# elasticdeeplearning/trainingjob-operator

Measured on AMD Instinct MI355X. Metric: tokens_per_sec_llama3_8b, higher is better.
Workload: dtype bf16; 1 GPU; model=llama3-8b, global_batch=4, seq_len=4096, parallelism=dp1, micro_batch=2, grad_accum=2, checkpoint_activations=False

## Files before the change

trainingjob_operator_amd/ops/attention.py:

```python
from __future__ import annotations

import math
import os
from typing import Optional

import torch

from . import native


def _supported(q: torch.Tensor, k: torch.Tensor) -> bool:
    B, H, S, D = q.shape
    HKV = k.shape[1]
    return (q.dtype == torch.bfloat16 and D == 128
            and (S % 256 == 0 or (S % 64 == 0 and HKV == H))
            and q.stride(-1) == 1 and k.stride(-1) == 1
            and H % HKV == 0)


def _run_fwd(q, k, v, scale):
    B, H, S, D = q.shape
    HKV = k.shape[1]
    lib = native.load(require=True)
    out = torch.empty(B, H, S, D, dtype=torch.bfloat16, device=q.device)
    lse = torch.empty(B, H, S, dtype=torch.float32, device=q.device)
    rc = lib.attn_fwd(
        native.stream_ptr(), q.data_ptr(), k.data_ptr(), v.data_ptr(),
        out.data_ptr(), lse.data_ptr(),
        q.stride(0), q.stride(1), q.stride(2),
        k.stride(0), k.stride(1), k.stride(2),
        v.stride(0), v.stride(1), v.stride(2),
        B, H, HKV, S, scale)
    native.check_rc(rc, "attn_fwd", f"B={B} H={H} HKV={HKV} S={S}")
    return out, lse


class _NativeFlashAttention(torch.autograd.Function):
    @staticmethod
    def forward(ctx, q, k, v, scale):
        out, lse = _run_fwd(q, k, v, scale)
        ctx.save_for_backward(q, k, v, out, lse)
        ctx.scale = scale
        return out

    @staticmethod
    def backward(ctx, gout):
        q, k, v, out, lse = ctx.saved_tensors
        B, H, S, D = q.shape
        if S % 256 == 0 and os.environ.get("AITJ_ATTN_BWD") != "aten":
            return (*_native_backward(q, k, v, out, lse, gout, ctx.scale),
                    None)
        philox = torch.empty(0, dtype=torch.int64, device=q.device)
        dq, dk, dv = torch.ops.aten._scaled_dot_product_flash_attention_backward(
            gout.contiguous(), q, k, v, out, lse,
            None, None, S, S, 0.0, True,
            philox, philox, scale=ctx.scale)
        return dq, dk, dv, None


def _native_backward(q, k, v, out, lse, gout, scale):
    B, H, S, D = q.shape
    HKV = k.shape[1]
    lib = native.load(require=True)
    dout = gout.contiguous()
    delta = torch.empty(B, H, S, dtype=torch.float32, device=q.device)
    dq = torch.empty(B, H, S, D, dtype=torch.bfloat16, device=q.device)
    dk = torch.empty(B, HKV, S, D, dtype=torch.bfloat16, device=q.device)
    dv = torch.empty(B, HKV, S, D, dtype=torch.bfloat16, device=q.device)
    rc = lib.attn_bwd(
        native.stream_ptr(), q.data_ptr(), k.data_ptr(), v.data_ptr(),
        out.data_ptr(), dout.data_ptr(), lse.data_ptr(), delta.data_ptr(),
        dq.data_ptr(), dk.data_ptr(), dv.data_ptr(),
        q.stride(0), q.stride(1), q.stride(2),
        k.stride(0), k.stride(1), k.stride(2),
        v.stride(0), v.stride(1), v.stride(2),
        B, H, HKV, S, scale)
    native.check_rc(rc, "attn_bwd", f"B={B} H={H} HKV={HKV} S={S}")
    return dq, dk, dv


def flash_attention(q: torch.Tensor, k: torch.Tensor, v: torch.Tensor,
                    scale: Optional[float] = None) -> torch.Tensor:
    if scale is None:
        scale = 1.0 / math.sqrt(q.shape[-1])
    assert _supported(q, k), (
        f"native flash attention needs bf16, D=128, S%256==0 (or S%64==0 "
        f"with equal head counts), d-contiguous strides; got {q.shape} "
        f"{q.dtype} kv={k.shape}")
    return _NativeFlashAttention.apply(q, k, v, scale)



def _bhsd_strides(row: int, D: int, S: int):
    return (S * row, D, row)


def _rope_packed(lib, x, out, inv_freq, n_tokens, n_rot, x_row, out_row,
                 S, D, sign):
    assert inv_freq.device == x.device and inv_freq.dtype == torch.float32, (
        f"inv_freq must be fp32 on {x.device}, got "
        f"{inv_freq.dtype}@{inv_freq.device}")
    rc = lib.rope_packed(native.stream_ptr(), x.data_ptr(), out.data_ptr(),
                         inv_freq.data_ptr(), n_tokens, n_rot, x_row,
                         out_row, S, D, sign)
    native.check_rc(rc, "rope_packed", f"D={D} n_rot={n_rot} row={x_row}")


class _PackedRopeAttention(torch.autograd.Function):

    @staticmethod
    def forward(ctx, qkv, inv_freq, n_heads, n_kv_heads, scale):
        B, S, W = qkv.shape
        D = 128
        H, HKV = n_heads, n_kv_heads
        assert W == (H + 2 * HKV) * D
        qkv = qkv.contiguous()
        lib = native.load(require=True)
        R = (H + HKV) * D
        rot = torch.empty(B, S, R, dtype=torch.bfloat16, device=qkv.device)
        _rope_packed(lib, qkv, rot, inv_freq, B * S, H + HKV, W, R, S, D, 1.0)
        o = torch.empty(B, S, H * D, dtype=torch.bfloat16, device=qkv.device)
        lse = torch.empty(B, H, S, dtype=torch.float32, device=qkv.device)
        esz = qkv.element_size()
        st = native.stride_array(
            _bhsd_strides(R, D, S), _bhsd_strides(R, D, S),
            _bhsd_strides(W, D, S), _bhsd_strides(H * D, D, S))
        rc = lib.attn_fwd_strided(
            native.stream_ptr(), rot.data_ptr(),
            rot.data_ptr() + H * D * esz,
            qkv.data_ptr() + (H + HKV) * D * esz,
            o.data_ptr(), lse.data_ptr(), st, B, H, HKV, S, scale)
        native.check_rc(rc, "attn_fwd_strided", f"B={B} H={H} HKV={HKV} S={S}")
        ctx.save_for_backward(rot, qkv, o, lse, inv_freq)
        ctx.dims = (B, S, H, HKV, D)
        ctx.scale = scale
        return o

    @staticmethod
    def backward(ctx, gout):
        rot, qkv, o, lse, inv_freq = ctx.saved_tensors
        B, S, H, HKV, D = ctx.dims
        W, R = (H + 2 * HKV) * D, (H + HKV) * D
        lib = native.load(require=True)
        dout = gout if gout.is_contiguous() else gout.contiguous()
        delta = torch.empty(B, H, S, dtype=torch.float32, device=qkv.device)
        dqkv = torch.empty(B, S, W, dtype=torch.bfloat16, device=qkv.device)
        esz = qkv.element_size()
        rs, ws, os_ = (_bhsd_strides(R, D, S), _bhsd_strides(W, D, S),
                       _bhsd_strides(H * D, D, S))
        st = native.stride_array(rs, rs, ws, os_, os_, ws, ws, ws)
        rc = lib.attn_bwd_strided(
            native.stream_ptr(), rot.data_ptr(),
            rot.data_ptr() + H * D * esz,
            qkv.data_ptr() + (H + HKV) * D * esz,
            o.data_ptr(), dout.data_ptr(), lse.data_ptr(), delta.data_ptr(),
            dqkv.data_ptr(), dqkv.data_ptr() + H * D * esz,
            dqkv.data_ptr() + (H + HKV) * D * esz,
            st, B, H, HKV, S, ctx.scale)
        native.check_rc(rc, "attn_bwd_strided", f"B={B} H={H} HKV={HKV} S={S}")
        _rope_packed(lib, dqkv, dqkv, inv_freq, B * S, H + HKV, W, W, S, D,
                     -1.0)
        return dqkv, None, None, None, None


def packed_supported(qkv: torch.Tensor, n_heads: int, n_kv_heads: int) -> bool:
    return (qkv.is_cuda and qkv.dtype == torch.bfloat16 and qkv.dim() == 3
            and qkv.shape[1] % 256 == 0 and n_heads % n_kv_heads == 0
            and qkv.shape[2] == (n_heads + 2 * n_kv_heads) * 128)


def unpacked_rope_attention(qkv, inv_freq, n_heads, n_kv_heads, scale=None):
    from .functional import apply_rope
    B, S, W = qkv.shape
    D = W // (n_heads + 2 * n_kv_heads)
    q, k, v = qkv.split([n_heads * D, n_kv_heads * D, n_kv_heads * D], dim=-1)
    q = q.reshape(B, S, n_heads, D).contiguous()
    k = k.reshape(B, S, n_kv_heads, D).contiguous()
    v = v.reshape(B, S, n_kv_heads, D)
    q = apply_rope(q, inv_freq, S).transpose(1, 2)
    k = apply_rope(k, inv_freq, S).transpose(1, 2)
    v = v.transpose(1, 2)
    if qkv.is_cuda and _supported(q, k):
        o = flash_attention(q, k, v, scale)
    else:
        o = torch.nn.functional.scaled_dot_product_attention(
            q, k, v, is_causal=True, scale=scale,
            enable_gqa=n_heads != n_kv_heads)
    return o.transpose(1, 2).reshape(B, S, n_heads * D)


def packed_rope_attention(qkv: torch.Tensor, inv_freq: torch.Tensor,
                          n_heads: int, n_kv_heads: int,
                          scale: Optional[float] = None) -> torch.Tensor:
    if packed_supported(qkv, n_heads, n_kv_heads):
        if scale is None:
            scale = 1.0 / math.sqrt(128)
        return _PackedRopeAttention.apply(qkv, inv_freq, n_heads, n_kv_heads,
                                          scale)
    return unpacked_rope_attention(qkv, inv_freq, n_heads, n_kv_heads, scale)


def flash_attention_fwd_only(q, k, v, scale=None):
    if scale is None:
        scale = 1.0 / math.sqrt(q.shape[-1])
    return _run_fwd(q, k, v, scale)


def flash_attention_fwd_nw8(q, k, v, scale=None):
    if scale is None:
        scale = 1.0 / math.sqrt(q.shape[-1])
    B, H, S, D = q.shape
    HKV = k.shape[1]
    lib = native.load(require=True)
    out = torch.empty(B, H, S, D, dtype=torch.bfloat16, device=q.device)
    lse = torch.empty(B, H, S, dtype=torch.float32, device=q.device)
    rc = lib.attn_fwd_nw8(
        native.stream_ptr(), q.data_ptr(), k.data_ptr(), v.data_ptr(),
        out.data_ptr(), lse.data_ptr(),
        q.stride(0), q.stride(1), q.stride(2),
        k.stride(0), k.stride(1), k.stride(2),
        v.stride(0), v.stride(1), v.stride(2),
        B, H, HKV, S, scale)
    native.check_rc(rc, "attn_fwd_nw8", f"B={B} H={H} S={S}")
    return out, lse


def flash_attention_fwd_v7(q, k, v, scale=None):
    if scale is None:
        scale = 1.0 / math.sqrt(q.shape[-1])
    B, H, S, D = q.shape
    HKV = k.shape[1]
    lib = native.load(require=True)
    out = torch.empty(B, H, S, D, dtype=torch.bfloat16, device=q.device)
    lse = torch.empty(B, H, S, dtype=torch.float32, device=q.device)
    rc = lib.attn_fwd_v7(
        native.stream_ptr(), q.data_ptr(), k.data_ptr(), v.data_ptr(),
        out.data_ptr(), lse.data_ptr(),
        q.stride(0), q.stride(1), q.stride(2),
        k.stride(0), k.stride(1), k.stride(2),
        v.stride(0), v.stride(1), v.stride(2),
        B, H, HKV, S, scale)
    native.check_rc(rc, "attn_fwd_v7", f"B={B} H={H} S={S}")
    return out, lse


def flash_attention_fwd_v5(q, k, v, scale=None):
    if scale is None:
        scale = 1.0 / math.sqrt(q.shape[-1])
    B, H, S, D = q.shape
    lib = native.load(require=True)
    out = torch.empty(B, H, S, D, dtype=torch.bfloat16, device=q.device)
    lse = torch.empty(B, H, S, dtype=torch.float32, device=q.device)
    rc = lib.attn_fwd_v5(
        native.stream_ptr(), q.data_ptr(), k.data_ptr(), v.data_ptr(),
        out.data_ptr(), lse.data_ptr(),
        q.stride(0), q.stride(1), q.stride(2),
        k.stride(0), k.stride(1), k.stride(2),
        v.stride(0), v.stride(1), v.stride(2),
        B, H, S, scale)
    native.check_rc(rc, "attn_fwd_v5", f"B={B} H={H} S={S}")
    return out, lse



def block_supported(q: torch.Tensor, k: torch.Tensor) -> bool:
    if q.dim() != 4 or k.dim() != 4:
        return False
    B, H, S, D = q.shape
    HKV = k.shape[1]
    return (q.is_cuda and k.is_cuda and q.dtype == torch.bfloat16
            and k.dtype == torch.bfloat16 and D == 128 and k.shape[-1] == 128
            and S % 256 == 0 and k.shape[2] == S and H % HKV == 0
            and q.stride(-1) == 1 and k.stride(-1) == 1)


def _tri(t: torch.Tensor):
    assert t.stride(-1) == 1, f"last stride must be 1, got {t.stride()}"
    return (t.stride(0), t.stride(1), t.stride(2))


def _block_dims(q, k, v, op):
    assert block_supported(q, k) and v.shape == k.shape \
        and v.dtype == q.dtype and v.is_cuda, (
            f"{op} needs GPU bf16 [B,H,S,128] / [B,HKV,S,128] with "
            f"S%256==0; got q {tuple(q.shape)} {q.dtype} "
            f"kv {tuple(k.shape)} {tuple(v.shape)}")
    B, H, S, _ = q.shape
    return B, H, k.shape[1], S


def flash_attention_block_fwd(q, k, v, causal: bool,
                              scale: Optional[float] = None):
    if scale is None:
        scale = 1.0 / math.sqrt(q.shape[-1])
    B, H, HKV, S = _block_dims(q, k, v, "flash_attention_block_fwd")
    lib = native.load(require=True)
    out = torch.empty(B, H, S, 128, dtype=torch.bfloat16, device=q.device)
    lse = torch.empty(B, H, S, dtype=torch.float32, device=q.device)
    st = native.stride_array(_tri(q), _tri(k), _tri(v), _tri(out))
    rc = lib.attn_block_fwd(
        native.stream_ptr(), q.data_ptr(), k.data_ptr(), v.data_ptr(),
        out.data_ptr(), lse.data_ptr(), st, B, H, HKV, S, scale,
        1 if causal else 0)
    native.check_rc(rc, "attn_block_fwd", f"B={B} H={H} HKV={HKV} S={S}")
    return out, lse


def flash_attention_delta(out: torch.Tensor,
                          dout: torch.Tensor) -> torch.Tensor:
    assert (out.is_cuda and out.dtype == torch.bfloat16
            and dout.dtype == torch.bfloat16 and out.shape == dout.shape
            and out.dim() == 4 and out.shape[-1] == 128
            and out.shape[2] % 16 == 0), (out.shape, out.dtype, dout.dtype)
    B, H, S, _ = out.shape
    lib = native.load(require=True)
    delta = torch.empty(B, H, S, dtype=torch.float32, device=out.device)
    st = native.stride_array(_tri(out), _tri(dout))
    rc = lib.attn_delta(native.stream_ptr(), out.data_ptr(), dout.data_ptr(),
                        delta.data_ptr(), st, B, H, S)
    native.check_rc(rc, "attn_delta", f"B={B} H={H} S={S}")
    return delta


def flash_attention_block_bwd(q, k, v, dout, lse, delta, causal: bool,
                              scale: Optional[float] = None):
    if scale is None:
        scale = 1.0 / math.sqrt(q.shape[-1])
    B, H, HKV, S = _block_dims(q, k, v, "flash_attention_block_bwd")
    assert dout.shape == q.shape and dout.dtype == torch.bfloat16
    assert lse.shape == (B, H, S) and delta.shape == (B, H, S)
    assert lse.dtype == torch.float32 and delta.dtype == torch.float32
    lib = native.load(require=True)
    if dout.stride(-1) != 1:
        dout = dout.contiguous()
    lse, delta = lse.contiguous(), delta.contiguous()
    dq = torch.empty(B, H, S, 128, dtype=torch.bfloat16, device=q.device)
    dk = torch.empty(B, HKV, S, 128, dtype=torch.bfloat16, device=q.device)
    dv = torch.empty(B, HKV, S, 128, dtype=torch.bfloat16, device=q.device)
    st = native.stride_array(_tri(q), _tri(k), _tri(v), _tri(dout),
                             _tri(dq), _tri(dk), _tri(dv))
    rc = lib.attn_block_bwd(
        native.stream_ptr(), q.data_ptr(), k.data_ptr(), v.data_ptr(),
        dout.data_ptr(), lse.data_ptr(), delta.data_ptr(),
        dq.data_ptr(), dk.data_ptr(), dv.data_ptr(), st,
        B, H, HKV, S, scale, 1 if causal else 0)
    native.check_rc(rc, "attn_block_bwd", f"B={B} H={H} HKV={HKV} S={S}")
    return dq, dk, dv


def attn_merge_(o_acc, lse_acc, o_blk, lse_blk) -> None:
    B, H, S, D = o_acc.shape
    assert (o_acc.is_cuda and D == 128 and o_acc.dtype == torch.float32
            and lse_acc.dtype == torch.float32
            and lse_blk.dtype == torch.float32
            and o_blk.dtype == torch.bfloat16
            and o_acc.is_contiguous() and lse_acc.is_contiguous()
            and o_blk.shape == o_acc.shape
            and lse_acc.shape == (B, H, S) and lse_blk.shape == (B, H, S)), (
        o_acc.shape, o_acc.dtype, o_blk.shape, o_blk.dtype, lse_acc.shape,
        lse_blk.shape)
    lib = native.load(require=True)
    lse_blk = lse_blk.contiguous()
    st = native.stride_array(_tri(o_blk))
    rc = lib.attn_merge(native.stream_ptr(), o_acc.data_ptr(),
                        lse_acc.data_ptr(), o_blk.data_ptr(),
                        lse_blk.data_ptr(), st, B, H, S)
    native.check_rc(rc, "attn_merge", f"B={B} H={H} S={S}")
```

trainingjob_operator_amd/ops/hip/attention.hip:

```cpp

#include <hip/hip_runtime.h>
#include <hip/hip_bf16.h>
#include <cstdint>

typedef unsigned short u16;
typedef unsigned int u32;
typedef __attribute__((ext_vector_type(8))) __bf16 bf16x8;
typedef __attribute__((ext_vector_type(4))) float f32x4;

#define ATTN_BM 64
#define ATTN_BN 64
#define ATTN_D 128
#define ATTN_WAVES 4
__device__ __forceinline__ u16 attn_f2bf(float f) {
  __hip_bfloat16_raw r = __float2bfloat16(f);
  return r.x;
}

__device__ __forceinline__ float bf2f_(u16 b) {
  union { u32 u; float f; } c;
  c.u = ((u32)b) << 16;
  return c.f;
}

__device__ __forceinline__ int k_byte(int row, int col_elem) {
  return (row * ATTN_D * 2 + col_elem * 2) ^ ((row & 15) << 4);
}

#define VT_PITCH_B 144
__device__ __forceinline__ int vt_byte(int d, int kv) {
  const int m = d >> 3;
  return (d * VT_PITCH_B + kv * 2) ^
         ((((m & 7) | (((m >> 1) & 1) << 3))) << 4);
}

__device__ __forceinline__ int p_byte(int row, int col_elem) {
  return (row * ATTN_BN * 2 + col_elem * 2) ^ ((row & 7) << 4);
}

__global__ __launch_bounds__(256) void attn_fwd_kernel(
    const u16* __restrict__ q, const u16* __restrict__ k,
    const u16* __restrict__ v, u16* __restrict__ out,
    float* __restrict__ lse,
    long q_sb, long q_sh, long q_ss,
    long k_sb, long k_sh, long k_ss,
    long v_sb, long v_sh, long v_ss,
    int n_heads, int S, float scale) {
  const int qb = blockIdx.x;
  const int h = blockIdx.y;
  const int b = blockIdx.z;
  const int wid = threadIdx.x >> 6;
  const int lane = threadIdx.x & 63;
  const int low = lane & 15;
  const int kg = lane >> 4;

  __shared__ u16 ldsK[ATTN_BN * ATTN_D];
  __shared__ u16 ldsV[ATTN_D * (VT_PITCH_B / 2) + 128];
  __shared__ u16 ldsP[ATTN_WAVES][16 * ATTN_BN];

  const u16* qbase = q + (long)b * q_sb + (long)h * q_sh
                     + (long)(qb * ATTN_BM) * q_ss;
  union { bf16x8 v; uint4 u; } qfrag[4];
#pragma unroll
  for (int ks = 0; ks < 4; ++ks) {
    qfrag[ks].u = *reinterpret_cast<const uint4*>(
        qbase + (long)(wid * 16 + low) * q_ss + ks * 32 + kg * 8);
  }

  float m_run[4], l_run[4];
  float oacc[8][4];
#pragma unroll
  for (int r = 0; r < 4; ++r) { m_run[r] = -INFINITY; l_run[r] = 0.f; }
#pragma unroll
  for (int ct = 0; ct < 8; ++ct)
#pragma unroll
    for (int r = 0; r < 4; ++r) oacc[ct][r] = 0.f;

  const u16* kbase = k + (long)b * k_sb + (long)h * k_sh;
  const u16* vbase = v + (long)b * v_sb + (long)h * v_sh;
  const int kv_end = (qb + 1) * ATTN_BM;
  char* ldsKb = reinterpret_cast<char*>(ldsK);
  char* ldsVb = reinterpret_cast<char*>(ldsV);
  char* ldsPb = reinterpret_cast<char*>(ldsP[wid]);

  for (int kv0 = 0; kv0 < kv_end; kv0 += ATTN_BN) {
#pragma unroll
    for (int t = 0; t < 4; ++t) {
      const int idx = t * 256 + threadIdx.x;
      const int r = idx >> 4;
      const int c8 = (idx & 15) * 8;
      *reinterpret_cast<uint4*>(&ldsKb[k_byte(r, c8)]) =
          *reinterpret_cast<const uint4*>(
              kbase + (long)(kv0 + r) * k_ss + c8);
      union { uint4 u; u16 h[8]; } vv;
      vv.u = *reinterpret_cast<const uint4*>(
          vbase + (long)(kv0 + r) * v_ss + c8);
#pragma unroll
      for (int j = 0; j < 8; ++j)
        *reinterpret_cast<u16*>(&ldsVb[vt_byte(c8 + j, r)]) = vv.h[j];
    }
    __syncthreads();

    f32x4 sacc[4];
#pragma unroll
    for (int ct = 0; ct < 4; ++ct) {
      f32x4 acc = {0.f, 0.f, 0.f, 0.f};
#pragma unroll
      for (int ks = 0; ks < 4; ++ks) {
        bf16x8 bfrag = *reinterpret_cast<const bf16x8*>(
            &ldsKb[k_byte(ct * 16 + low, ks * 32 + kg * 8)]);
        acc = __builtin_amdgcn_mfma_f32_16x16x32_bf16(qfrag[ks].v, bfrag,
                                                      acc, 0, 0, 0);
      }
      sacc[ct] = acc;
    }

    const int qrow0 = qb * ATTN_BM + wid * 16 + kg * 4;
    float mx[4], alpha[4], psum[4];
#pragma unroll
    for (int r = 0; r < 4; ++r) {
      mx[r] = -INFINITY;
#pragma unroll
      for (int ct = 0; ct < 4; ++ct) {
        const int col = kv0 + ct * 16 + low;
        float s = sacc[ct][r] * scale;
        if (col > qrow0 + r) s = -INFINITY;
        sacc[ct][r] = s;
        mx[r] = fmaxf(mx[r], s);
      }
#pragma unroll
      for (int off = 1; off < 16; off <<= 1)
        mx[r] = fmaxf(mx[r], __shfl_xor(mx[r], off, 64));
      const float mnew = fmaxf(m_run[r], mx[r]);
      alpha[r] = (m_run[r] == -INFINITY) ? 0.f : __expf(m_run[r] - mnew);
      m_run[r] = mnew;
      psum[r] = 0.f;
#pragma unroll
      for (int ct = 0; ct < 4; ++ct) {
        const float p = (sacc[ct][r] == -INFINITY)
                            ? 0.f : __expf(sacc[ct][r] - mnew);
        sacc[ct][r] = p;
        psum[r] += p;
        *reinterpret_cast<u16*>(
            &ldsPb[p_byte(kg * 4 + r, ct * 16 + low)]) = attn_f2bf(p);
      }
#pragma unroll
      for (int off = 1; off < 16; off <<= 1)
        psum[r] += __shfl_xor(psum[r], off, 64);
      l_run[r] = l_run[r] * alpha[r] + psum[r];
#pragma unroll
      for (int ct2 = 0; ct2 < 8; ++ct2) oacc[ct2][r] *= alpha[r];
    }
    __syncthreads();

#pragma unroll
    for (int ct2 = 0; ct2 < 8; ++ct2) {
      f32x4 acc = {oacc[ct2][0], oacc[ct2][1], oacc[ct2][2], oacc[ct2][3]};
#pragma unroll
      for (int ks2 = 0; ks2 < 2; ++ks2) {
        bf16x8 afrag = *reinterpret_cast<const bf16x8*>(
            &ldsPb[p_byte(low, ks2 * 32 + kg * 8)]);
        bf16x8 bfrag = *reinterpret_cast<const bf16x8*>(
            &ldsVb[vt_byte(ct2 * 16 + low, ks2 * 32 + kg * 8)]);
        acc = __builtin_amdgcn_mfma_f32_16x16x32_bf16(afrag, bfrag, acc,
                                                      0, 0, 0);
      }
#pragma unroll
      for (int r = 0; r < 4; ++r) oacc[ct2][r] = acc[r];
    }
    __syncthreads();
  }

  u16* obase = out + (((long)b * n_heads + h) * S + qb * ATTN_BM
                      + wid * 16) * ATTN_D;
#pragma unroll
  for (int r = 0; r < 4; ++r) {
    const float inv_l = 1.0f / l_run[r];
#pragma unroll
    for (int ct2 = 0; ct2 < 8; ++ct2) {
      obase[(long)(kg * 4 + r) * ATTN_D + ct2 * 16 + low] =
          attn_f2bf(oacc[ct2][r] * inv_l);
    }
  }
  if (low == 0) {
    float* lbase = lse + ((long)b * n_heads + h) * S + qb * ATTN_BM
                   + wid * 16 + kg * 4;
#pragma unroll
    for (int r = 0; r < 4; ++r) lbase[r] = m_run[r] + __logf(l_run[r]);
  }
}


typedef __attribute__((ext_vector_type(16))) float f32x16;

#define V6_BM 256
#define V6_QBLK 32
#define V6_BN 64
#define V6_K_U16 (V6_BN * ATTN_D)
#define V6_V_U16 (ATTN_D * (VT_PITCH_B / 2) + 128)
#define V6_BUF_U16 (V6_K_U16 + V6_V_U16)

__device__ __forceinline__ unsigned cvt_pk_bf16(float lo, float hi) {
  unsigned r;
  asm("v_cvt_pk_bf16_f32 %0, %1, %2" : "=v"(r) : "v"(lo), "v"(hi));
  return r;
}

__device__ __forceinline__ float exp2_raw(float x) {
  float r;
  asm("v_exp_f32 %0, %1" : "=v"(r) : "v"(x));
  return r;
}

__device__ __forceinline__ void v7_wait_vmcnt4() {
  asm volatile("s_waitcnt vmcnt(4)" ::: "memory");
}
__device__ __forceinline__ void v7_wait_vmcnt0() {
  asm volatile("s_waitcnt vmcnt(0)" ::: "memory");
}
__device__ __forceinline__ void v7_barrier() {
  asm volatile("s_waitcnt lgkmcnt(0)" ::: "memory");
  __builtin_amdgcn_s_barrier();
}

#define V7_RING 3


template <int NW>
__global__ __launch_bounds__(NW * 64) void attn_fwd_v6_kernel(
    const u16* __restrict__ q, const u16* __restrict__ k,
    const u16* __restrict__ v, u16* __restrict__ out,
    float* __restrict__ lse,
    long q_sb, long q_sh, long q_ss,
    long k_sb, long k_sh, long k_ss,
    long v_sb, long v_sh, long v_ss,
    int n_heads, int gqa_group, int S, float scale2) {
  constexpr int NT = NW * 64;
  constexpr int BM = NW * 32;
  constexpr int KP = 1024 / NT;
  constexpr int VU = 512 / NT;
  const int qb = gridDim.x - 1 - blockIdx.x;
  const int h = blockIdx.y;
  const int b = blockIdx.z;
  const int hkv = h / gqa_group;
  const int tid = threadIdx.x;
  const int wid = tid >> 6;
  const int lane = tid & 63;
  const int low = lane & 31;
  const int hi = lane >> 5;

  __shared__ __attribute__((aligned(16))) u16 lds[2][V6_BUF_U16];

  const int q0w = qb * BM + wid * V6_QBLK;
  const int qrow = q0w + low;

  union F8 { bf16x8 v; uint4 u; u16 h[8]; };
  const u16* qptr = q + (long)b * q_sb + (long)h * q_sh + (long)qrow * q_ss;
  F8 qf[8];
#pragma unroll
  for (int kc = 0; kc < 8; ++kc)
    qf[kc].u = *reinterpret_cast<const uint4*>(qptr + kc * 16 + hi * 8);

  f32x16 oacc[4];
#pragma unroll
  for (int ds = 0; ds < 4; ++ds)
#pragma unroll
    for (int r = 0; r < 16; ++r) oacc[ds][r] = 0.f;
  float m_run = -INFINITY, l_run = 0.f;

  const u16* kbase = k + (long)b * k_sb + (long)hkv * k_sh;
  const u16* vbase = v + (long)b * v_sb + (long)hkv * v_sh;
  const int n_tiles = (qb * BM + BM) / V6_BN;

  char* lds0 = reinterpret_cast<char*>(&lds[0][0]);
  char* lds1 = reinterpret_cast<char*>(&lds[1][0]);
  const int VOFF = V6_K_U16 * 2;

  const u16* kgp[KP];
  const u16* vgp[2 * VU];
#pragma unroll
  for (int i = 0; i < KP; ++i) {
    const int idx = i * NT + tid;
    const int L = idx * 16;
    const int kr = L >> 8;
    const int kin = (((L & 255) ^ ((kr & 15) << 4)) >> 1);
    kgp[i] = kbase + (long)kr * k_ss + kin;
  }
#pragma unroll
  for (int u = 0; u < VU; ++u) {
    const int unit = u * NT + tid;
    const int rp2 = (unit >> 4) * 2;
    const int c8 = (unit & 15) * 8;
#pragma unroll
    for (int i = 0; i < 2; ++i)
      vgp[u * 2 + i] = vbase + (long)(rp2 + i) * v_ss + c8;
  }
  const long kstep = (long)V6_BN * k_ss;
  const long vstep = (long)V6_BN * v_ss;
  const int wu64 = __builtin_amdgcn_readfirstlane(tid >> 6);

  uint4 vst[2 * VU];
#define V6_GLDS_K(BUFI)                                                     \
  _Pragma("unroll")                                                         \
  for (int i = 0; i < KP; ++i) {                                            \
    __builtin_amdgcn_global_load_lds(                                       \
        (const u32*)kgp[i], (u32*)&lds[BUFI][(i * NT + wu64 * 64) * 8],     \
        16, 0, 0);                                                          \
    kgp[i] += kstep;                                                        \
  }
#define V6_LOAD_V()                                                         \
  _Pragma("unroll")                                                         \
  for (int i = 0; i < 2 * VU; ++i) {                                        \
    vst[i] = *reinterpret_cast<const uint4*>(vgp[i]);                       \
    vgp[i] += vstep;                                                        \
  }
#define V6_WRITE_V(BUF)                                                     \
  _Pragma("unroll")                                                         \
  for (int u = 0; u < VU; ++u) {                                            \
    const int unit_ = u * NT + tid;                                         \
    const int rp2_ = (unit_ >> 4) * 2;                                      \
    const int c8_ = (unit_ & 15) * 8;                                       \
    union { uint4 u4; u16 h[8]; } va_, vb_;                                 \
    va_.u4 = vst[u * 2];                                                    \
    vb_.u4 = vst[u * 2 + 1];                                                \
    _Pragma("unroll")                                                       \
    for (int j = 0; j < 8; ++j) {                                           \
      const u32 pair_ = (u32)va_.h[j] | ((u32)vb_.h[j] << 16);              \
      *reinterpret_cast<u32*>(&(BUF)[VOFF + vt_byte(c8_ + j, rp2_)]) = pair_; \
    }                                                                       \
  }

  V6_GLDS_K(0)
  V6_LOAD_V()
  V6_WRITE_V(lds0)
  __syncthreads();

  if (NW == 8 && __builtin_amdgcn_readfirstlane(threadIdx.x) >= NT / 2)
    __builtin_amdgcn_s_setprio(1);

  int cur = 0;
  for (int t = 0; t < n_tiles; ++t) {
    const int kv0 = t * V6_BN;
    const bool have_next = (t + 1) < n_tiles;
    if (have_next) { V6_GLDS_K(cur ^ 1) V6_LOAD_V() }

    char* kb = cur ? lds1 : lds0;
    char* vbuf = kb + VOFF;
    const bool active = kv0 <= q0w + V6_QBLK - 1;
    const bool need_mask = kv0 + V6_BN > q0w;

    f32x16 s0, s1;
    union PF { bf16x8 v; unsigned u[4]; } pa[4];
    float pm = -INFINITY;
    if (active) {
#pragma unroll
      for (int r = 0; r < 16; ++r) { s0[r] = 0.f; s1[r] = 0.f; }
#pragma unroll
      for (int kc = 0; kc < 8; ++kc) {
        bf16x8 a0 = *reinterpret_cast<const bf16x8*>(
            &kb[k_byte(low, kc * 16 + hi * 8)]);
        s0 = __builtin_amdgcn_mfma_f32_32x32x16_bf16(a0, qf[kc].v, s0, 0, 0, 0);
        bf16x8 a1 = *reinterpret_cast<const bf16x8*>(
            &kb[k_byte(32 + low, kc * 16 + hi * 8)]);
        s1 = __builtin_amdgcn_mfma_f32_32x32x16_bf16(a1, qf[kc].v, s1, 0, 0, 0);
      }
      if (need_mask) {
#pragma unroll
        for (int r = 0; r < 16; ++r) {
          const int kvr = kv0 + (r & 3) + 8 * (r >> 2) + 4 * hi;
          float x0 = s0[r] * scale2;
          if (kvr > qrow) x0 = -1e30f;
          s0[r] = x0;
          float x1 = s1[r] * scale2;
          if (kvr + 32 > qrow) x1 = -1e30f;
          s1[r] = x1;
          pm = fmaxf(pm, fmaxf(x0, x1));
        }
      } else {
#pragma unroll
        for (int r = 0; r < 16; ++r) {
          s0[r] *= scale2;
          s1[r] *= scale2;
          pm = fmaxf(pm, fmaxf(s0[r], s1[r]));
        }
      }
      pm = fmaxf(pm, __shfl_xor(pm, 32, 64));
    }
    if (have_next) {
      char* nb = cur ? lds0 : lds1;
      V6_WRITE_V(nb)
    }
    if (active) {
      if (!__all(pm - m_run <= 8.0f)) {
        const float mn = fmaxf(m_run, pm);
        const float alpha = (m_run == -INFINITY) ? 0.f : exp2_raw(m_run - mn);
        m_run = mn;
        l_run *= alpha;
#pragma unroll
        for (int ds = 0; ds < 4; ++ds)
#pragma unroll
          for (int r = 0; r < 16; ++r) oacc[ds][r] *= alpha;
      }
      float psum = 0.f;
#pragma unroll
      for (int r = 0; r < 16; ++r) {
        const float p0 = exp2_raw(s0[r] - m_run);
        const float p1 = exp2_raw(s1[r] - m_run);
        s0[r] = p0;
        s1[r] = p1;
        psum += p0 + p1;
      }
      psum += __shfl_xor(psum, 32, 64);
      l_run += psum;

#pragma unroll
      for (int sub = 0; sub < 2; ++sub) {
#pragma unroll
        for (int cc = 0; cc < 2; ++cc) {
          const int pb = cc * 8;
          unsigned a0, b0, a1, b1;
          if (sub == 0) {
            a0 = cvt_pk_bf16(s0[pb + 0], s0[pb + 1]);
            b0 = cvt_pk_bf16(s0[pb + 4], s0[pb + 5]);
            a1 = cvt_pk_bf16(s0[pb + 2], s0[pb + 3]);
            b1 = cvt_pk_bf16(s0[pb + 6], s0[pb + 7]);
          } else {
            a0 = cvt_pk_bf16(s1[pb + 0], s1[pb + 1]);
            b0 = cvt_pk_bf16(s1[pb + 4], s1[pb + 5]);
            a1 = cvt_pk_bf16(s1[pb + 2], s1[pb + 3]);
            b1 = cvt_pk_bf16(s1[pb + 6], s1[pb + 7]);
          }
          auto r02 = __builtin_amdgcn_permlane32_swap(a0, b0, false, false);
          auto r13 = __builtin_amdgcn_permlane32_swap(a1, b1, false, false);
          PF f;
          f.u[0] = r02[0];
          f.u[1] = r13[0];
          f.u[2] = r02[1];
          f.u[3] = r13[1];
          pa[sub * 2 + cc] = f;
        }
      }

#pragma unroll
      for (int c = 0; c < 4; ++c) {
#pragma unroll
        for (int ds = 0; ds < 4; ++ds) {
          bf16x8 vf = *reinterpret_cast<const bf16x8*>(
              &vbuf[vt_byte(ds * 32 + low, c * 16 + hi * 8)]);
          oacc[ds] = __builtin_amdgcn_mfma_f32_32x32x16_bf16(
              vf, pa[c].v, oacc[ds], 0, 0, 0);
        }
      }
    }
    __syncthreads();
    cur ^= 1;
  }

  const float inv_l = 1.0f / l_run;
  u16* orow = out + (((long)b * n_heads + h) * S + qrow) * ATTN_D;
#pragma unroll
  for (int ds = 0; ds < 4; ++ds) {
#pragma unroll
    for (int g = 0; g < 4; ++g) {
      const int d0 = 8 * g + 4 * hi + 32 * ds;
      const unsigned w0 = cvt_pk_bf16(oacc[ds][4 * g + 0] * inv_l,
                                      oacc[ds][4 * g + 1] * inv_l);
      const unsigned w1 = cvt_pk_bf16(oacc[ds][4 * g + 2] * inv_l,
                                      oacc[ds][4 * g + 3] * inv_l);
      uint2 wv;
      wv.x = w0;
      wv.y = w1;
      *reinterpret_cast<uint2*>(orow + d0) = wv;
    }
  }
  if (hi == 0)
    lse[((long)b * n_heads + h) * S + qrow] =
        m_run * 0.6931471805599453f + __logf(l_run);
}

template <bool CAUSAL>
__global__ __launch_bounds__(512) void attn_fwd_v7_kernel(
    const u16* __restrict__ q, const u16* __restrict__ k,
    const u16* __restrict__ v, u16* __restrict__ out,
    float* __restrict__ lse,
    long q_sb, long q_sh, long q_ss,
    long k_sb, long k_sh, long k_ss,
    long v_sb, long v_sh, long v_ss,
    long o_sb, long o_sh, long o_ss,
    int n_heads, int gqa_group, int S, float scale2);

static inline bool attn_strides_ok(const long* st, int n) {
  for (int i = 0; i < n; ++i)
    if (st[i] < 0 || st[i] % 8 != 0) return false;
  return true;
}

static void launch_fwd_v7(void* stream, const void* q, const void* k,
                          const void* v, void* out, void* lse,
                          long q_sb, long q_sh, long q_ss,
                          long k_sb, long k_sh, long k_ss,
                          long v_sb, long v_sh, long v_ss,
                          long o_sb, long o_sh, long o_ss,
                          int batch, int n_heads, int n_kv_heads, int S,
                          float scale, bool causal = true) {
  const float scale2 = scale * 1.4426950408889634f;
  dim3 grid(S / 256, n_heads, batch), block(512);
  hipLaunchKernelGGL(causal ? attn_fwd_v7_kernel<true>
                            : attn_fwd_v7_kernel<false>, grid, block, 0,
                     reinterpret_cast<hipStream_t>(stream),
                     (const u16*)q, (const u16*)k, (const u16*)v,
                     (u16*)out, (float*)lse, q_sb, q_sh, q_ss,
                     k_sb, k_sh, k_ss, v_sb, v_sh, v_ss,
                     o_sb, o_sh, o_ss, n_heads,
                     n_heads / n_kv_heads, S, scale2);
}

extern "C" int attn_fwd(void* stream, const void* q, const void* k,
                        const void* v, void* out, void* lse,
                        long q_sb, long q_sh, long q_ss,
                        long k_sb, long k_sh, long k_ss,
                        long v_sb, long v_sh, long v_ss,
                        int batch, int n_heads, int n_kv_heads, int S,
                        float scale) {
  if (S <= 0 || n_heads <= 0 || batch <= 0 || n_kv_heads <= 0 ||
      n_heads % n_kv_heads != 0)
    return -1;
  if (S % 128 == 0) {
    const float scale2 = scale * 1.4426950408889634f;
    if (S % 256 == 0) {
      launch_fwd_v7(stream, q, k, v, out, lse, q_sb, q_sh, q_ss,
                    k_sb, k_sh, k_ss, v_sb, v_sh, v_ss,
                    (long)n_heads * S * ATTN_D, (long)S * ATTN_D, ATTN_D,
                    batch, n_heads, n_kv_heads, S, scale);
      return 0;
    }
    dim3 grid(S / 128, n_heads, batch), block(256);
    hipLaunchKernelGGL((attn_fwd_v6_kernel<4>), grid, block, 0,
                       reinterpret_cast<hipStream_t>(stream),
                       (const u16*)q, (const u16*)k, (const u16*)v, (u16*)out,
                       (float*)lse, q_sb, q_sh, q_ss, k_sb, k_sh, k_ss,
                       v_sb, v_sh, v_ss, n_heads, n_heads / n_kv_heads, S,
                       scale2);
    return 0;
  }
  if (S % ATTN_BM != 0 || n_kv_heads != n_heads) return -1;
  dim3 grid(S / ATTN_BM, n_heads, batch), block(256);
  hipLaunchKernelGGL(attn_fwd_kernel, grid, block, 0,
                     reinterpret_cast<hipStream_t>(stream),
                     (const u16*)q, (const u16*)k, (const u16*)v, (u16*)out,
                     (float*)lse, q_sb, q_sh, q_ss, k_sb, k_sh, k_ss,
                     v_sb, v_sh, v_ss, n_heads, S, scale);
  return 0;
}

extern "C" int attn_fwd_nw8(void* stream, const void* q, const void* k,
                            const void* v, void* out, void* lse,
                            long q_sb, long q_sh, long q_ss,
                            long k_sb, long k_sh, long k_ss,
                            long v_sb, long v_sh, long v_ss,
                            int batch, int n_heads, int n_kv_heads, int S,
                            float scale) {
  if (S <= 0 || S % 256 != 0 || n_heads % n_kv_heads != 0) return -1;
  dim3 grid(S / 256, n_heads, batch), block(512);
  const float scale2 = scale * 1.4426950408889634f;
  hipLaunchKernelGGL((attn_fwd_v6_kernel<8>), grid, block, 0,
                     reinterpret_cast<hipStream_t>(stream),
                     (const u16*)q, (const u16*)k, (const u16*)v, (u16*)out,
                     (float*)lse, q_sb, q_sh, q_ss, k_sb, k_sh, k_ss,
                     v_sb, v_sh, v_ss, n_heads, n_heads / n_kv_heads, S,
                     scale2);
  return 0;
}

extern "C" int attn_fwd_v5(void* stream, const void* q, const void* k,
                           const void* v, void* out, void* lse,
                           long q_sb, long q_sh, long q_ss,
                           long k_sb, long k_sh, long k_ss,
                           long v_sb, long v_sh, long v_ss,
                           int batch, int n_heads, int S, float scale) {
  if (S <= 0 || S % ATTN_BM != 0 || n_heads <= 0 || batch <= 0) return -1;
  dim3 grid(S / ATTN_BM, n_heads, batch), block(256);
  hipLaunchKernelGGL(attn_fwd_kernel, grid, block, 0,
                     reinterpret_cast<hipStream_t>(stream),
                     (const u16*)q, (const u16*)k, (const u16*)v, (u16*)out,
                     (float*)lse, q_sb, q_sh, q_ss, k_sb, k_sh, k_ss,
                     v_sb, v_sh, v_ss, n_heads, S, scale);
  return 0;
}


__global__ __launch_bounds__(256) void attn_delta_kernel(
    const u16* __restrict__ dout, const u16* __restrict__ o,
    float* __restrict__ delta,
    long do_sb, long do_sh, long do_ss,
    long o_sb, long o_sh, long o_ss,
    int n_heads, int S) {
  const int s = blockIdx.x * 16 + (threadIdx.x >> 4);
  const int h = blockIdx.y;
  const int bi = blockIdx.z;
  if (s >= S) return;
  const long row = ((long)bi * n_heads + h) * S + s;
  const int e8 = (threadIdx.x & 15) * 8;
  union { uint4 u; u16 h[8]; } a, b;
  a.u = *reinterpret_cast<const uint4*>(
      dout + (long)bi * do_sb + (long)h * do_sh + (long)s * do_ss + e8);
  b.u = *reinterpret_cast<const uint4*>(
      o + (long)bi * o_sb + (long)h * o_sh + (long)s * o_ss + e8);
  float acc = 0.f;
#pragma unroll
  for (int j = 0; j < 8; ++j)
    acc += bf2f_(a.h[j]) * bf2f_(b.h[j]);
#pragma unroll
  for (int off = 1; off < 16; off <<= 1) acc += __shfl_xor(acc, off, 64);
  if ((threadIdx.x & 15) == 0) delta[row] = acc;
}


#define BQ_K_U16 (V6_BN * ATTN_D)
#define BQ_KT_U16 (ATTN_D * (VT_PITCH_B / 2) + 128)
#define BQ_V_U16 (V6_BN * ATTN_D)
#define BQ_BUF_U16 (BQ_K_U16 + BQ_KT_U16 + BQ_V_U16)

template <bool CAUSAL>
__global__ __launch_bounds__(512) void attn_bwd_dq_kernel(
    const u16* __restrict__ q, const u16* __restrict__ k,
    const u16* __restrict__ v, const u16* __restrict__ dout,
    const float* __restrict__ lse, const float* __restrict__ delta,
    u16* __restrict__ dq,
    long q_sb, long q_sh, long q_ss,
    long k_sb, long k_sh, long k_ss,
    long v_sb, long v_sh, long v_ss,
    long do_sb, long do_sh, long do_ss,
    long dq_sb, long dq_sh, long dq_ss,
    int n_heads, int gqa_group, int S, float scale) {
  constexpr int NT = 512;
  const int qb = gridDim.x - 1 - blockIdx.x;
  const int h = blockIdx.y;
  const int b = blockIdx.z;
  const int hkv = h / gqa_group;
  const int tid = threadIdx.x;
  const int wid = tid >> 6;
  const int lane = tid & 63;
  const int low = lane & 31;
  const int hi = lane >> 5;
  const float scale2 = scale * 1.4426950408889634f;

  __shared__ __attribute__((aligned(16))) u16
      lds[V7_RING * 2 * V6_K_U16 + 2 * V6_V_U16];
#define DQ_K(SLOT) (&lds[(SLOT) * V6_K_U16])
#define DQ_VR(SLOT) (&lds[(V7_RING + (SLOT)) * V6_K_U16])
#define DQ_KT(P) (reinterpret_cast<char*>(&lds[2 * V7_RING * V6_K_U16]) \
                  + (P) * (V6_V_U16 * 2))

  const int q0w = qb * 256 + wid * 32;
  const int qrow = q0w + low;

  union F8 { bf16x8 v; uint4 u; u16 h[8]; };
  const u16* qptr = q + (long)b * q_sb + (long)h * q_sh + (long)qrow * q_ss;
  const u16* doptr = dout + (long)b * do_sb + (long)h * do_sh
                     + (long)qrow * do_ss;
  F8 qf[8], dof[8];
#pragma unroll
  for (int kc = 0; kc < 8; ++kc) {
    qf[kc].u = *reinterpret_cast<const uint4*>(qptr + kc * 16 + hi * 8);
    dof[kc].u = *reinterpret_cast<const uint4*>(doptr + kc * 16 + hi * 8);
  }
  const long lrow = ((long)b * n_heads + h) * S + qrow;
  const float lse2 = lse[lrow] * 1.4426950408889634f;
  const float dlt = delta[lrow];

  f32x16 dqacc[4];
#pragma unroll
  for (int ds = 0; ds < 4; ++ds)
#pragma unroll
    for (int r = 0; r < 16; ++r) dqacc[ds][r] = 0.f;

  const u16* kbase = k + (long)b * k_sb + (long)hkv * k_sh;
  const u16* vbase = v + (long)b * v_sb + (long)hkv * v_sh;
  const int n_tiles = CAUSAL ? (qb + 1) * 4 : S / V6_BN;

  const u16* kgp[2];
  const u16* vgp[2];
#pragma unroll
  for (int i = 0; i < 2; ++i) {
    const int L = (tid & ~63) * 32 + i * 1024 + (tid & 63) * 16;
    const int kr = L >> 8;
    const int kin = (((L & 255) ^ ((kr & 15) << 4)) >> 1);
    kgp[i] = kbase + (long)kr * k_ss + kin;
    vgp[i] = vbase + (long)kr * v_ss + kin;
  }
  const long kstep = (long)V6_BN * k_ss;
  const long vstep = (long)V6_BN * v_ss;
  const int lslot = (tid & ~63) * 16;

#define DQ_GLDS(SLOT)                                                       \
  _Pragma("unroll")                                                         \
  for (int i = 0; i < 2; ++i) {                                             \
    __builtin_amdgcn_global_load_lds(                                       \
        (const u32*)kgp[i], (u32*)&DQ_K(SLOT)[i * 512 + lslot],          \
        16, 0, 0);                                                          \
    kgp[i] += kstep;                                                        \
    __builtin_amdgcn_global_load_lds(                                       \
        (const u32*)vgp[i], (u32*)&DQ_VR(SLOT)[i * 512 + lslot],         \
        16, 0, 0);                                                          \
    vgp[i] += vstep;                                                        \
  }

  const int t_rp2 = (tid >> 4) * 2;
  const int t_c8 = (tid & 15) * 8;
#define DQ_TRANSPOSE(SRCSLOT, DST)                                          \
  {                                                                         \
    const char* srcb = reinterpret_cast<const char*>(DQ_K(SRCSLOT));        \
    union { uint4 u4; u16 h[8]; } va_, vb_;                                 \
    va_.u4 = *reinterpret_cast<const uint4*>(&srcb[k_byte(t_rp2, t_c8)]);   \
    vb_.u4 = *reinterpret_cast<const uint4*>(                               \
        &srcb[k_byte(t_rp2 + 1, t_c8)]);                                    \
    _Pragma("unroll")                                                       \
    for (int j = 0; j < 8; ++j) {                                           \
      const u32 pair_ = (u32)va_.h[j] | ((u32)vb_.h[j] << 16);              \
      *reinterpret_cast<u32*>(&(DST)[vt_byte(t_c8 + j, t_rp2)]) = pair_;    \
    }                                                                       \
  }

  DQ_GLDS(0)
  if (n_tiles > 1) DQ_GLDS(1)
  if (n_tiles > 1) v7_wait_vmcnt4(); else v7_wait_vmcnt0();
  v7_barrier();
  DQ_TRANSPOSE(0, DQ_KT(0))
  v7_barrier();

  for (int t = 0; t < n_tiles; ++t) {
    const int kv0 = t * V6_BN;
    const bool have2 = (t + 2) < n_tiles;
    if (have2) DQ_GLDS((t + 2) % V7_RING)

    char* kb = reinterpret_cast<char*>(DQ_K(t % V7_RING));
    char* vb = reinterpret_cast<char*>(DQ_VR(t % V7_RING));
    char* ktb = DQ_KT(t & 1);
    const bool active = !CAUSAL || kv0 <= q0w + 31;
    const bool need_mask = CAUSAL && kv0 + V6_BN > q0w;

    union PF { bf16x8 v; unsigned u[4]; } pds[4];
    if (active) {
#pragma unroll
      for (int sub = 0; sub < 2; ++sub) {
        f32x16 sx, dp;
#pragma unroll
        for (int r = 0; r < 16; ++r) { sx[r] = 0.f; dp[r] = 0.f; }
#pragma unroll
        for (int kc = 0; kc < 8; ++kc) {
          bf16x8 a = *reinterpret_cast<const bf16x8*>(
              &kb[k_byte(sub * 32 + low, kc * 16 + hi * 8)]);
          sx = __builtin_amdgcn_mfma_f32_32x32x16_bf16(a, qf[kc].v, sx,
                                                       0, 0, 0);
          bf16x8 a2 = *reinterpret_cast<const bf16x8*>(
              &vb[k_byte(sub * 32 + low, kc * 16 + hi * 8)]);
          dp = __builtin_amdgcn_mfma_f32_32x32x16_bf16(a2, dof[kc].v, dp,
                                                       0, 0, 0);
        }
#pragma unroll
        for (int r = 0; r < 16; ++r) {
          float x = sx[r] * scale2 - lse2;
          if (need_mask) {
            const int kvr = kv0 + sub * 32 + (r & 3) + 8 * (r >> 2) + 4 * hi;
            if (kvr > qrow) x = -1e30f;
          }
          const float p = exp2_raw(x);
          sx[r] = p * (dp[r] - dlt) * scale;
        }
#pragma unroll
        for (int cc = 0; cc < 2; ++cc) {
          const int pb = cc * 8;
          unsigned a0 = cvt_pk_bf16(sx[pb + 0], sx[pb + 1]);
          unsigned b0 = cvt_pk_bf16(sx[pb + 4], sx[pb + 5]);
          unsigned a1 = cvt_pk_bf16(sx[pb + 2], sx[pb + 3]);
          unsigned b1 = cvt_pk_bf16(sx[pb + 6], sx[pb + 7]);
          auto r02 = __builtin_amdgcn_permlane32_swap(a0, b0, false, false);
          auto r13 = __builtin_amdgcn_permlane32_swap(a1, b1, false, false);
          PF f;
          f.u[0] = r02[0];
          f.u[1] = r13[0];
          f.u[2] = r02[1];
          f.u[3] = r13[1];
          pds[sub * 2 + cc] = f;
        }
      }
#pragma unroll
      for (int c = 0; c < 4; ++c) {
#pragma unroll
        for (int ds = 0; ds < 4; ++ds) {
          bf16x8 kf = *reinterpret_cast<const bf16x8*>(
              &ktb[vt_byte(ds * 32 + low, c * 16 + hi * 8)]);
          dqacc[ds] = __builtin_amdgcn_mfma_f32_32x32x16_bf16(
              kf, pds[c].v, dqacc[ds], 0, 0, 0);
        }
      }
    }
    if (t + 1 < n_tiles) {
      if (have2) v7_wait_vmcnt4(); else v7_wait_vmcnt0();
      DQ_TRANSPOSE((t + 1) % V7_RING, DQ_KT((t + 1) & 1))
    }
    v7_barrier();
  }

  u16* dqrow = dq + (long)b * dq_sb + (long)h * dq_sh + (long)qrow * dq_ss;
#pragma unroll
  for (int ds = 0; ds < 4; ++ds) {
#pragma unroll
    for (int g = 0; g < 4; ++g) {
      const int d0 = 8 * g + 4 * hi + 32 * ds;
      const unsigned w0 = cvt_pk_bf16(dqacc[ds][4 * g + 0],
                                      dqacc[ds][4 * g + 1]);
      const unsigned w1 = cvt_pk_bf16(dqacc[ds][4 * g + 2],
                                      dqacc[ds][4 * g + 3]);
      uint2 wv;
      wv.x = w0;
      wv.y = w1;
      *reinterpret_cast<uint2*>(dqrow + d0) = wv;
    }
  }
}


#define BV_Q_U16 (V6_BN * ATTN_D)
#define BV_DOT_U16 (ATTN_D * (VT_PITCH_B / 2) + 128)
#define BV_LSE_U16 128
#define BV_BUF_U16 (BV_Q_U16 + BV_DOT_U16 + BV_LSE_U16)

template <bool CAUSAL>
__global__ __launch_bounds__(512) void attn_bwd_dv_kernel(
    const u16* __restrict__ q, const u16* __restrict__ k,
    const u16* __restrict__ dout, const float* __restrict__ lse,
    u16* __restrict__ dv,
    long q_sb, long q_sh, long q_ss,
    long k_sb, long k_sh, long k_ss,
    long do_sb, long do_sh, long do_ss,
    long dv_sb, long dv_sh, long dv_ss,
    int n_heads, int n_kv_heads, int S, float scale) {
  const int kvb = blockIdx.x;
  const int hkv = blockIdx.y;
  const int b = blockIdx.z;
  const int gqa_group = n_heads / n_kv_heads;
  const int tid = threadIdx.x;
  const int wid = tid >> 6;
  const int lane = tid & 63;
  const int low = lane & 31;
  const int hi = lane >> 5;
  const float scale2 = scale * 1.4426950408889634f;

  __shared__ __attribute__((aligned(16))) u16 lds[2][BV_BUF_U16];
  char* lds0 = reinterpret_cast<char*>(&lds[0][0]);
  char* lds1 = reinterpret_cast<char*>(&lds[1][0]);
  const int DOTOFF = BV_Q_U16 * 2;
  const int LSEOFF = (BV_Q_U16 + BV_DOT_U16) * 2;

  const int kv0w = kvb * 256 + wid * 32;
  const int kvrow = kv0w + low;

  union F8 { bf16x8 v; uint4 u; u16 h[8]; };
  const u16* kptr = k + (long)b * k_sb + (long)hkv * k_sh + (long)kvrow * k_ss;
  F8 kf[8];
#pragma unroll
  for (int kc = 0; kc < 8; ++kc)
    kf[kc].u = *reinterpret_cast<const uint4*>(kptr + kc * 16 + hi * 8);

  f32x16 dvacc[4];
#pragma unroll
  for (int ds = 0; ds < 4; ++ds)
#pragma unroll
    for (int r = 0; r < 16; ++r) dvacc[ds][r] = 0.f;

  const int qt0 = CAUSAL ? kvb * 4 : 0;
  const int qtn = S / 64;
  const int wu64 = __builtin_amdgcn_readfirstlane(tid >> 6);
  uint4 dtst[2];

  for (int g = 0; g < gqa_group; ++g) {
    const int h = hkv * gqa_group + g;
    const u16* qbase = q + (long)b * q_sb + (long)h * q_sh;
    const u16* dobase = dout + (long)b * do_sb + (long)h * do_sh;
    const float* lbase = lse + ((long)b * n_heads + h) * S;

    const u16* qgp[2];
    const u16* dtp[2];
    {
      const int idx0 = tid, idx1 = 512 + tid;
      const int L0 = idx0 * 16, L1 = idx1 * 16;
      const int r0 = L0 >> 8, r1 = L1 >> 8;
      const int in0 = (((L0 & 255) ^ ((r0 & 15) << 4)) >> 1);
      const int in1 = (((L1 & 255) ^ ((r1 & 15) << 4)) >> 1);
      qgp[0] = qbase + (long)(qt0 * 64 + r0) * q_ss + in0;
      qgp[1] = qbase + (long)(qt0 * 64 + r1) * q_ss + in1;
      const int rp2 = (tid >> 4) * 2;
      const int c8 = (tid & 15) * 8;
      dtp[0] = dobase + (long)(qt0 * 64 + rp2) * do_ss + c8;
      dtp[1] = dobase + (long)(qt0 * 64 + rp2 + 1) * do_ss + c8;
    }
    const long qstep = (long)64 * q_ss;
    const long dostep = (long)64 * do_ss;

#define BV_STAGE_IN(BUFI, QT)                                               \
    {                                                                       \
      _Pragma("unroll")                                                     \
      for (int i = 0; i < 2; ++i) {                                         \
        __builtin_amdgcn_global_load_lds(                                   \
            (const u32*)qgp[i], (u32*)&lds[BUFI][(i * 512 + wu64 * 64) * 8],\
            16, 0, 0);                                                      \
        qgp[i] += qstep;                                                    \
      }                                                                     \
      dtst[0] = *reinterpret_cast<const uint4*>(dtp[0]);                    \
      dtst[1] = *reinterpret_cast<const uint4*>(dtp[1]);                    \
      dtp[0] += dostep;                                                     \
      dtp[1] += dostep;                                                     \
      if (tid < 64)                                                         \
        *reinterpret_cast<float*>(                                          \
            &lds[BUFI][LSEOFF / 2 + tid * 2]) =                             \
            lbase[(QT) * 64 + tid] * 1.4426950408889634f;                   \
    }
#define BV_WRITE_DOT(BUF)                                                   \
    {                                                                       \
      const int rp2_ = (tid >> 4) * 2;                                      \
      const int c8_ = (tid & 15) * 8;                                       \
      union { uint4 u4; u16 h[8]; } va_, vb_;                               \
      va_.u4 = dtst[0];                                                     \
      vb_.u4 = dtst[1];                                                     \
      _Pragma("unroll")                                                     \
      for (int j = 0; j < 8; ++j) {                                         \
        const u32 pair_ = (u32)va_.h[j] | ((u32)vb_.h[j] << 16);            \
        *reinterpret_cast<u32*>(&(BUF)[DOTOFF + vt_byte(c8_ + j, rp2_)]) =  \
            pair_;                                                          \
      }                                                                     \
    }

    BV_STAGE_IN(0, qt0)
    BV_WRITE_DOT(lds0)
    __syncthreads();

    int cur = 0;
    for (int qt = qt0; qt < qtn; ++qt) {
      const bool have_next = (qt + 1) < qtn;
      if (have_next) BV_STAGE_IN(cur ^ 1, qt + 1)

      char* qb_ = cur ? lds1 : lds0;
      char* dob = qb_ + DOTOFF;
      const float* lse2t = reinterpret_cast<const float*>(qb_ + LSEOFF);
      const bool active = !CAUSAL || qt * 64 + 63 >= kv0w;
      const bool need_mask = CAUSAL && qt * 64 < kv0w + 32;

      union PF { bf16x8 v; unsigned u[4]; } pf[4];
      if (active) {
#pragma unroll
        for (int sub = 0; sub < 2; ++sub) {
          f32x16 s;
#pragma unroll
          for (int r = 0; r < 16; ++r) s[r] = 0.f;
#pragma unroll
          for (int kc = 0; kc < 8; ++kc) {
            bf16x8 a = *reinterpret_cast<const bf16x8*>(
                &qb_[k_byte(sub * 32 + low, kc * 16 + hi * 8)]);
            s = __builtin_amdgcn_mfma_f32_32x32x16_bf16(a, kf[kc].v, s,
                                                        0, 0, 0);
          }
#pragma unroll
          for (int r = 0; r < 16; ++r) {
            const int qr = (r & 3) + 8 * (r >> 2) + 4 * hi;
            float x = s[r] * scale2 - lse2t[sub * 32 + qr];
            if (need_mask && qt * 64 + sub * 32 + qr < kvrow) x = -1e30f;
            s[r] = exp2_raw(x);
          }
#pragma unroll
          for (int cc = 0; cc < 2; ++cc) {
            const int pb = cc * 8;
            unsigned a0 = cvt_pk_bf16(s[pb + 0], s[pb + 1]);
            unsigned b0 = cvt_pk_bf16(s[pb + 4], s[pb + 5]);
            unsigned a1 = cvt_pk_bf16(s[pb + 2], s[pb + 3]);
            unsigned b1 = cvt_pk_bf16(s[pb + 6], s[pb + 7]);
            auto r02 = __builtin_amdgcn_permlane32_swap(a0, b0, false, false);
            auto r13 = __builtin_amdgcn_permlane32_swap(a1, b1, false, false);
            PF f;
            f.u[0] = r02[0];
            f.u[1] = r13[0];
            f.u[2] = r02[1];
            f.u[3] = r13[1];
            pf[sub * 2 + cc] = f;
          }
        }
      }
      if (have_next) {
        char* nb = cur ? lds0 : lds1;
        BV_WRITE_DOT(nb)
      }
      if (active) {
#pragma unroll
        for (int c = 0; c < 4; ++c) {
#pragma unroll
          for (int ds = 0; ds < 4; ++ds) {
            bf16x8 af = *reinterpret_cast<const bf16x8*>(
                &dob[vt_byte(ds * 32 + low, c * 16 + hi * 8)]);
            dvacc[ds] = __builtin_amdgcn_mfma_f32_32x32x16_bf16(
                af, pf[c].v, dvacc[ds], 0, 0, 0);
          }
        }
      }
      __syncthreads();
      cur ^= 1;
    }
  }

  u16* dvrow = dv + (long)b * dv_sb + (long)hkv * dv_sh + (long)kvrow * dv_ss;
#pragma unroll
  for (int ds = 0; ds < 4; ++ds) {
#pragma unroll
    for (int g = 0; g < 4; ++g) {
      const int d0 = 8 * g + 4 * hi + 32 * ds;
      const unsigned w0 = cvt_pk_bf16(dvacc[ds][4 * g + 0],
                                      dvacc[ds][4 * g + 1]);
      const unsigned w1 = cvt_pk_bf16(dvacc[ds][4 * g + 2],
                                      dvacc[ds][4 * g + 3]);
      uint2 wv;
      wv.x = w0;
      wv.y = w1;
      *reinterpret_cast<uint2*>(dvrow + d0) = wv;
    }
  }
}


#define BK_Q_U16 (V6_BN * ATTN_D)
#define BK_DO_U16 (V6_BN * ATTN_D)
#define BK_QT_U16 (ATTN_D * (VT_PITCH_B / 2) + 128)
#define BK_LSE_U16 128
#define BK_DLT_U16 128
#define BK_BUF_U16 (BK_Q_U16 + BK_DO_U16 + BK_QT_U16 + BK_LSE_U16 + BK_DLT_U16)

template <bool CAUSAL>
__global__ __launch_bounds__(512) void attn_bwd_dk_kernel(
    const u16* __restrict__ q, const u16* __restrict__ k,
    const u16* __restrict__ v, const u16* __restrict__ dout,
    const float* __restrict__ lse, const float* __restrict__ delta,
    u16* __restrict__ dk,
    long q_sb, long q_sh, long q_ss,
    long k_sb, long k_sh, long k_ss,
    long v_sb, long v_sh, long v_ss,
    long do_sb, long do_sh, long do_ss,
    long dk_sb, long dk_sh, long dk_ss,
    int n_heads, int n_kv_heads, int S, float scale) {
  const int kvb = blockIdx.x;
  const int hkv = blockIdx.y;
  const int b = blockIdx.z;
  const int gqa_group = n_heads / n_kv_heads;
  const int tid = threadIdx.x;
  const int wid = tid >> 6;
  const int lane = tid & 63;
  const int low = lane & 31;
  const int hi = lane >> 5;
  const float scale2 = scale * 1.4426950408889634f;

  __shared__ __attribute__((aligned(16))) u16 lds[2][BK_BUF_U16];
  char* lds0 = reinterpret_cast<char*>(&lds[0][0]);
  char* lds1 = reinterpret_cast<char*>(&lds[1][0]);
  const int DOOFF = BK_Q_U16 * 2;
  const int QTOFF = (BK_Q_U16 + BK_DO_U16) * 2;
  const int LSEOFF = (BK_Q_U16 + BK_DO_U16 + BK_QT_U16) * 2;
  const int DLTOFF = LSEOFF + BK_LSE_U16 * 2;

  const int kv0w = kvb * 256 + wid * 32;
  const int kvrow = kv0w + low;

  union F8 { bf16x8 v; uint4 u; u16 h[8]; };
  const u16* kptr = k + (long)b * k_sb + (long)hkv * k_sh + (long)kvrow * k_ss;
  const u16* vptr = v + (long)b * v_sb + (long)hkv * v_sh + (long)kvrow * v_ss;
  F8 kf[8], vf[8];
#pragma unroll
  for (int kc = 0; kc < 8; ++kc) {
    kf[kc].u = *reinterpret_cast<const uint4*>(kptr + kc * 16 + hi * 8);
    vf[kc].u = *reinterpret_cast<const uint4*>(vptr + kc * 16 + hi * 8);
  }

  f32x16 dkacc[4];
#pragma unroll
  for (int ds = 0; ds < 4; ++ds)
#pragma unroll
    for (int r = 0; r < 16; ++r) dkacc[ds][r] = 0.f;

  const int qt0 = CAUSAL ? kvb * 4 : 0;
  const int qtn = S / 64;
  const int wu64 = __builtin_amdgcn_readfirstlane(tid >> 6);
  uint4 qtst[2];

  for (int g = 0; g < gqa_group; ++g) {
    const int h = hkv * gqa_group + g;
    const u16* qbase = q + (long)b * q_sb + (long)h * q_sh;
    const u16* dobase = dout + (long)b * do_sb + (long)h * do_sh;
    const float* lbase = lse + ((long)b * n_heads + h) * S;
    const float* dbase = delta + ((long)b * n_heads + h) * S;

    const u16* qgp[2];
    const u16* dgp[2];
    const u16* qtp[2];
    {
      const int idx0 = tid, idx1 = 512 + tid;
      const int L0 = idx0 * 16, L1 = idx1 * 16;
      const int r0 = L0 >> 8, r1 = L1 >> 8;
      const int in0 = (((L0 & 255) ^ ((r0 & 15) << 4)) >> 1);
      const int in1 = (((L1 & 255) ^ ((r1 & 15) << 4)) >> 1);
      qgp[0] = qbase + (long)(qt0 * 64 + r0) * q_ss + in0;
      qgp[1] = qbase + (long)(qt0 * 64 + r1) * q_ss + in1;
      dgp[0] = dobase + (long)(qt0 * 64 + r0) * do_ss + in0;
      dgp[1] = dobase + (long)(qt0 * 64 + r1) * do_ss + in1;
      const int rp2 = (tid >> 4) * 2;
      const int c8 = (tid & 15) * 8;
      qtp[0] = qbase + (long)(qt0 * 64 + rp2) * q_ss + c8;
      qtp[1] = qbase + (long)(qt0 * 64 + rp2 + 1) * q_ss + c8;
    }
    const long qstep = (long)64 * q_ss;
    const long dostep = (long)64 * do_ss;

#define BK_STAGE_IN(BUFI, QT)                                               \
    {                                                                       \
      _Pragma("unroll")                                                     \
      for (int i = 0; i < 2; ++i) {                                         \
        __builtin_amdgcn_global_load_lds(                                   \
            (const u32*)qgp[i], (u32*)&lds[BUFI][(i * 512 + wu64 * 64) * 8],\
            16, 0, 0);                                                      \
        qgp[i] += qstep;                                                    \
        __builtin_amdgcn_global_load_lds(                                   \
            (const u32*)dgp[i],                                             \
            (u32*)&lds[BUFI][DOOFF / 2 + (i * 512 + wu64 * 64) * 8],        \
            16, 0, 0);                                                      \
        dgp[i] += dostep;                                                   \
      }                                                                     \
      qtst[0] = *reinterpret_cast<const uint4*>(qtp[0]);                    \
      qtst[1] = *reinterpret_cast<const uint4*>(qtp[1]);                    \
      qtp[0] += qstep;                                                      \
      qtp[1] += qstep;                                                      \
      if (tid < 64)                                                         \
        *reinterpret_cast<float*>(&lds[BUFI][LSEOFF / 2 + tid * 2]) =       \
            lbase[(QT) * 64 + tid] * 1.4426950408889634f;                   \
      else if (tid < 128)                                                   \
        *reinterpret_cast<float*>(                                          \
            &lds[BUFI][DLTOFF / 2 + (tid - 64) * 2]) =                      \
            dbase[(QT) * 64 + tid - 64];                                    \
    }
#define BK_WRITE_QT(BUF)                                                    \
    {                                                                       \
      const int rp2_ = (tid >> 4) * 2;                                      \
      const int c8_ = (tid & 15) * 8;                                       \
      union { uint4 u4; u16 h[8]; } va_, vb_;                               \
      va_.u4 = qtst[0];                                                     \
      vb_.u4 = qtst[1];                                                     \
      _Pragma("unroll")                                                     \
      for (int j = 0; j < 8; ++j) {                                         \
        const u32 pair_ = (u32)va_.h[j] | ((u32)vb_.h[j] << 16);            \
        *reinterpret_cast<u32*>(&(BUF)[QTOFF + vt_byte(c8_ + j, rp2_)]) =   \
            pair_;                                                          \
      }                                                                     \
    }

    BK_STAGE_IN(0, qt0)
    BK_WRITE_QT(lds0)
    __syncthreads();

    int cur = 0;
    for (int qt = qt0; qt < qtn; ++qt) {
      const bool have_next = (qt + 1) < qtn;
      if (have_next) BK_STAGE_IN(cur ^ 1, qt + 1)

      char* qb_ = cur ? lds1 : lds0;
      char* dob = qb_ + DOOFF;
      char* qtb = qb_ + QTOFF;
      const float* lse2t = reinterpret_cast<const float*>(qb_ + LSEOFF);
      const float* dltt = reinterpret_cast<const float*>(qb_ + DLTOFF);
      const bool active = !CAUSAL || qt * 64 + 63 >= kv0w;
      const bool need_mask = CAUSAL && qt * 64 < kv0w + 32;

      union PF { bf16x8 v; unsigned u[4]; } pf[4];
      if (active) {
#pragma unroll
        for (int sub = 0; sub < 2; ++sub) {
          f32x16 s, dp;
#pragma unroll
          for (int r = 0; r < 16; ++r) { s[r] = 0.f; dp[r] = 0.f; }
#pragma unroll
          for (int kc = 0; kc < 8; ++kc) {
            bf16x8 a = *reinterpret_cast<const bf16x8*>(
                &qb_[k_byte(sub * 32 + low, kc * 16 + hi * 8)]);
            s = __builtin_amdgcn_mfma_f32_32x32x16_bf16(a, kf[kc].v, s,
                                                        0, 0, 0);
            bf16x8 a2 = *reinterpret_cast<const bf16x8*>(
                &dob[k_byte(sub * 32 + low, kc * 16 + hi * 8)]);
            dp = __builtin_amdgcn_mfma_f32_32x32x16_bf16(a2, vf[kc].v, dp,
                                                         0, 0, 0);
          }
#pragma unroll
          for (int r = 0; r < 16; ++r) {
            const int qr = (r & 3) + 8 * (r >> 2) + 4 * hi;
            float x = s[r] * scale2 - lse2t[sub * 32 + qr];
            if (need_mask && qt * 64 + sub * 32 + qr < kvrow) x = -1e30f;
            const float p = exp2_raw(x);
            s[r] = p * (dp[r] - dltt[sub * 32 + qr]) * scale;
          }
#pragma unroll
          for (int cc = 0; cc < 2; ++cc) {
            const int pb = cc * 8;
            unsigned a0 = cvt_pk_bf16(s[pb + 0], s[pb + 1]);
            unsigned b0 = cvt_pk_bf16(s[pb + 4], s[pb + 5]);
            unsigned a1 = cvt_pk_bf16(s[pb + 2], s[pb + 3]);
            unsigned b1 = cvt_pk_bf16(s[pb + 6], s[pb + 7]);
            auto r02 = __builtin_amdgcn_permlane32_swap(a0, b0, false, false);
            auto r13 = __builtin_amdgcn_permlane32_swap(a1, b1, false, false);
            PF f;
            f.u[0] = r02[0];
            f.u[1] = r13[0];
            f.u[2] = r02[1];
            f.u[3] = r13[1];
            pf[sub * 2 + cc] = f;
          }
        }
      }
      if (have_next) {
        char* nb = cur ? lds0 : lds1;
        BK_WRITE_QT(nb)
      }
      if (active) {
#pragma unroll
        for (int c = 0; c < 4; ++c) {
#pragma unroll
          for (int ds = 0; ds < 4; ++ds) {
            bf16x8 af = *reinterpret_cast<const bf16x8*>(
                &qtb[vt_byte(ds * 32 + low, c * 16 + hi * 8)]);
            dkacc[ds] = __builtin_amdgcn_mfma_f32_32x32x16_bf16(
                af, pf[c].v, dkacc[ds], 0, 0, 0);
          }
        }
      }
      __syncthreads();
      cur ^= 1;
    }
  }

  u16* dkrow = dk + (long)b * dk_sb + (long)hkv * dk_sh + (long)kvrow * dk_ss;
#pragma unroll
  for (int ds = 0; ds < 4; ++ds) {
#pragma unroll
    for (int g = 0; g < 4; ++g) {
      const int d0 = 8 * g + 4 * hi + 32 * ds;
      const unsigned w0 = cvt_pk_bf16(dkacc[ds][4 * g + 0],
                                      dkacc[ds][4 * g + 1]);
      const unsigned w1 = cvt_pk_bf16(dkacc[ds][4 * g + 2],
                                      dkacc[ds][4 * g + 3]);
      uint2 wv;
      wv.x = w0;
      wv.y = w1;
      *reinterpret_cast<uint2*>(dkrow + d0) = wv;
    }
  }
}




struct AttnStride { long sb, sh, ss; };

static inline AttnStride attn_dense_stride(int n_heads, int S) {
  return {(long)n_heads * S * ATTN_D, (long)S * ATTN_D, (long)ATTN_D};
}

static void launch_delta(hipStream_t st, const void* out, const void* dout,
                         void* delta, AttnStride os, AttnStride dos,
                         int batch, int n_heads, int S) {
  hipLaunchKernelGGL(attn_delta_kernel, dim3(S / 16, n_heads, batch),
                     dim3(256), 0, st,
                     (const u16*)dout, (const u16*)out, (float*)delta,
                     dos.sb, dos.sh, dos.ss, os.sb, os.sh, os.ss,
                     n_heads, S);
}

template <bool CAUSAL>
static void launch_bwd_core(hipStream_t st, const void* q, const void* k,
                            const void* v, const void* dout,
                            const void* lse, const void* delta,
                            void* dq, void* dk, void* dv,
                            AttnStride qs, AttnStride ks, AttnStride vs,
                            AttnStride dos, AttnStride dqs, AttnStride dks,
                            AttnStride dvs, int batch, int n_heads,
                            int n_kv_heads, int S, float scale) {
  {
    dim3 grid(S / 256, n_heads, batch), block(512);
    hipLaunchKernelGGL(attn_bwd_dq_kernel<CAUSAL>, grid, block, 0, st,
                       (const u16*)q, (const u16*)k, (const u16*)v,
                       (const u16*)dout, (const float*)lse,
                       (const float*)delta, (u16*)dq,
                       qs.sb, qs.sh, qs.ss, ks.sb, ks.sh, ks.ss,
                       vs.sb, vs.sh, vs.ss, dos.sb, dos.sh, dos.ss,
                       dqs.sb, dqs.sh, dqs.ss,
                       n_heads, n_heads / n_kv_heads, S, scale);
  }
  {
    dim3 grid(S / 256, n_kv_heads, batch), block(512);
    hipLaunchKernelGGL(attn_bwd_dv_kernel<CAUSAL>, grid, block, 0, st,
                       (const u16*)q, (const u16*)k, (const u16*)dout,
                       (const float*)lse, (u16*)dv,
                       qs.sb, qs.sh, qs.ss, ks.sb, ks.sh, ks.ss,
                       dos.sb, dos.sh, dos.ss, dvs.sb, dvs.sh, dvs.ss,
                       n_heads, n_kv_heads, S, scale);
    hipLaunchKernelGGL(attn_bwd_dk_kernel<CAUSAL>, grid, block, 0, st,
                       (const u16*)q, (const u16*)k, (const u16*)v,
                       (const u16*)dout, (const float*)lse,
                       (const float*)delta, (u16*)dk,
                       qs.sb, qs.sh, qs.ss, ks.sb, ks.sh, ks.ss,
                       vs.sb, vs.sh, vs.ss, dos.sb, dos.sh, dos.ss,
                       dks.sb, dks.sh, dks.ss,
                       n_heads, n_kv_heads, S, scale);
  }
}

static inline bool attn_block_shape_ok(int batch, int n_heads,
                                       int n_kv_heads, int S) {
  return S > 0 && S % 256 == 0 && n_heads > 0 && batch > 0 &&
         n_kv_heads > 0 && n_heads % n_kv_heads == 0;
}

static int launch_bwd(void* stream, const void* q, const void* k,
                      const void* v, const void* out, const void* dout,
                      const void* lse, void* delta,
                      void* dq, void* dk, void* dv,
                      AttnStride qs, AttnStride ks, AttnStride vs,
                      AttnStride os, AttnStride dos,
                      AttnStride dqs, AttnStride dks, AttnStride dvs,
                      int batch, int n_heads, int n_kv_heads, int S,
                      float scale) {
  if (!attn_block_shape_ok(batch, n_heads, n_kv_heads, S)) return -1;
  hipStream_t st = reinterpret_cast<hipStream_t>(stream);
  launch_delta(st, out, dout, delta, os, dos, batch, n_heads, S);
  launch_bwd_core<true>(st, q, k, v, dout, lse, delta, dq, dk, dv,
                        qs, ks, vs, dos, dqs, dks, dvs,
                        batch, n_heads, n_kv_heads, S, scale);
  return 0;
}

extern "C" int attn_bwd(void* stream, const void* q, const void* k,
                        const void* v, const void* out, const void* dout,
                        const void* lse, void* delta,
                        void* dq, void* dk, void* dv,
                        long q_sb, long q_sh, long q_ss,
                        long k_sb, long k_sh, long k_ss,
                        long v_sb, long v_sh, long v_ss,
                        int batch, int n_heads, int n_kv_heads, int S,
                        float scale) {
  const AttnStride dh = attn_dense_stride(n_heads, S);
  const AttnStride dkv = attn_dense_stride(n_kv_heads, S);
  return launch_bwd(stream, q, k, v, out, dout, lse, delta, dq, dk, dv,
                    {q_sb, q_sh, q_ss}, {k_sb, k_sh, k_ss},
                    {v_sb, v_sh, v_ss}, dh, dh, dh, dkv, dkv,
                    batch, n_heads, n_kv_heads, S, scale);
}

extern "C" int attn_bwd_strided(void* stream, const void* q, const void* k,
                                const void* v, const void* out,
                                const void* dout, const void* lse,
                                void* delta, void* dq, void* dk, void* dv,
                                const long* st, int batch, int n_heads,
                                int n_kv_heads, int S, float scale) {
  if (!st || !attn_strides_ok(st, 24)) return -1;
  auto tri = [st](int i) {
    return AttnStride{st[3 * i], st[3 * i + 1], st[3 * i + 2]};
  };
  return launch_bwd(stream, q, k, v, out, dout, lse, delta, dq, dk, dv,
                    tri(0), tri(1), tri(2), tri(3), tri(4), tri(5), tri(6),
                    tri(7), batch, n_heads, n_kv_heads, S, scale);
}


template <bool CAUSAL>
__global__ __launch_bounds__(512) void attn_fwd_v7_kernel(
    const u16* __restrict__ q, const u16* __restrict__ k,
    const u16* __restrict__ v, u16* __restrict__ out,
    float* __restrict__ lse,
    long q_sb, long q_sh, long q_ss,
    long k_sb, long k_sh, long k_ss,
    long v_sb, long v_sh, long v_ss,
    long o_sb, long o_sh, long o_ss,
    int n_heads, int gqa_group, int S, float scale2) {
  constexpr int NT = 512;
  const int qb = gridDim.x - 1 - blockIdx.x;
  const int h = blockIdx.y;
  const int b = blockIdx.z;
  const int hkv = h / gqa_group;
  const int tid = threadIdx.x;
  const int wid = tid >> 6;
  const int lane = tid & 63;
  const int low = lane & 31;
  const int hi = lane >> 5;

  __shared__ __attribute__((aligned(16))) u16
      lds[V7_RING * 2 * V6_K_U16 + 2 * V6_V_U16];
#define LDSK(SLOT) (&lds[(SLOT) * V6_K_U16])
#define LDSVR(SLOT) (&lds[(V7_RING + (SLOT)) * V6_K_U16])
#define LDSVT(P) (reinterpret_cast<char*>(&lds[2 * V7_RING * V6_K_U16]) \
                  + (P) * (V6_V_U16 * 2))

  const int q0w = qb * 256 + wid * 32;
  const int qrow = q0w + low;

  union F8 { bf16x8 v; uint4 u; u16 h[8]; };
  const u16* qptr = q + (long)b * q_sb + (long)h * q_sh + (long)qrow * q_ss;
  F8 qf[8];
#pragma unroll
  for (int kc = 0; kc < 8; ++kc)
    qf[kc].u = *reinterpret_cast<const uint4*>(qptr + kc * 16 + hi * 8);

  f32x16 oacc[4];
#pragma unroll
  for (int ds = 0; ds < 4; ++ds)
#pragma unroll
    for (int r = 0; r < 16; ++r) oacc[ds][r] = 0.f;
  float m_run = -INFINITY, l_run = 0.f;

  const u16* kbase = k + (long)b * k_sb + (long)hkv * k_sh;
  const u16* vbase = v + (long)b * v_sb + (long)hkv * v_sh;
  const int n_tiles = CAUSAL ? (qb + 1) * 4 : S / V6_BN;

  const u16* kgp[2];
  const u16* vgp[2];
#pragma unroll
  for (int i = 0; i < 2; ++i) {
    const int L = (tid & ~63) * 32 + i * 1024 + (tid & 63) * 16;
    const int kr = L >> 8;
    const int kin = (((L & 255) ^ ((kr & 15) << 4)) >> 1);
    kgp[i] = kbase + (long)kr * k_ss + kin;
    vgp[i] = vbase + (long)kr * v_ss + kin;
  }
  const long kstep = (long)V6_BN * k_ss;
  const long vstep = (long)V6_BN * v_ss;
  const int lslot = (tid & ~63) * 16;

#define V7_GLDS(SLOT)                                                       \
  _Pragma("unroll")                                                         \
  for (int i = 0; i < 2; ++i) {                                             \
    __builtin_amdgcn_global_load_lds(                                       \
        (const u32*)kgp[i], (u32*)&LDSK(SLOT)[i * 512 + lslot],          \
        16, 0, 0);                                                          \
    kgp[i] += kstep;                                                        \
    __builtin_amdgcn_global_load_lds(                                       \
        (const u32*)vgp[i], (u32*)&LDSVR(SLOT)[i * 512 + lslot],         \
        16, 0, 0);                                                          \
    vgp[i] += vstep;                                                        \
  }

  const int t_rp2 = (tid >> 4) * 2;
  const int t_c8 = (tid & 15) * 8;
#define V7_TRANSPOSE(SRCSLOT, DST)                                          \
  {                                                                         \
    const char* srcb = reinterpret_cast<const char*>(LDSVR(SRCSLOT));       \
    union { uint4 u4; u16 h[8]; } va_, vb_;                                 \
    va_.u4 = *reinterpret_cast<const uint4*>(&srcb[k_byte(t_rp2, t_c8)]);   \
    vb_.u4 = *reinterpret_cast<const uint4*>(                               \
        &srcb[k_byte(t_rp2 + 1, t_c8)]);                                    \
    _Pragma("unroll")                                                       \
    for (int j = 0; j < 8; ++j) {                                           \
      const u32 pair_ = (u32)va_.h[j] | ((u32)vb_.h[j] << 16);              \
      *reinterpret_cast<u32*>(&(DST)[vt_byte(t_c8 + j, t_rp2)]) = pair_;    \
    }                                                                       \
  }

  V7_GLDS(0)
  if (n_tiles > 1) V7_GLDS(1)
  if (n_tiles > 1) v7_wait_vmcnt4(); else v7_wait_vmcnt0();
  v7_barrier();
  V7_TRANSPOSE(0, LDSVT(0))
  v7_barrier();

  for (int t = 0; t < n_tiles; ++t) {
    const int kv0 = t * V6_BN;
    const bool have2 = (t + 2) < n_tiles;
    if (have2) V7_GLDS((t + 2) % V7_RING)

    char* kb = reinterpret_cast<char*>(LDSK(t % V7_RING));
    char* vtb = LDSVT(t & 1);
    const bool active = !CAUSAL || kv0 <= q0w + 31;
    const bool need_mask = CAUSAL && kv0 + V6_BN > q0w;

    f32x16 s0, s1;
    union PF { bf16x8 v; unsigned u[4]; } pa[4];
    float pm = -INFINITY;
    if (active) {
#pragma unroll
      for (int r = 0; r < 16; ++r) { s0[r] = 0.f; s1[r] = 0.f; }
#pragma unroll
      for (int kc = 0; kc < 8; ++kc) {
        bf16x8 a0 = *reinterpret_cast<const bf16x8*>(
            &kb[k_byte(low, kc * 16 + hi * 8)]);
        s0 = __builtin_amdgcn_mfma_f32_32x32x16_bf16(a0, qf[kc].v, s0, 0, 0, 0);
        bf16x8 a1 = *reinterpret_cast<const bf16x8*>(
            &kb[k_byte(32 + low, kc * 16 + hi * 8)]);
        s1 = __builtin_amdgcn_mfma_f32_32x32x16_bf16(a1, qf[kc].v, s1, 0, 0, 0);
      }
      if (need_mask) {
#pragma unroll
        for (int r = 0; r < 16; ++r) {
          const int kvr = kv0 + (r & 3) + 8 * (r >> 2) + 4 * hi;
          float x0 = s0[r] * scale2;
          if (kvr > qrow) x0 = -1e30f;
          s0[r] = x0;
          float x1 = s1[r] * scale2;
          if (kvr + 32 > qrow) x1 = -1e30f;
          s1[r] = x1;
          pm = fmaxf(pm, fmaxf(x0, x1));
        }
      } else {
#pragma unroll
        for (int r = 0; r < 16; ++r) {
          s0[r] *= scale2;
          s1[r] *= scale2;
          pm = fmaxf(pm, fmaxf(s0[r], s1[r]));
        }
      }
      pm = fmaxf(pm, __shfl_xor(pm, 32, 64));

      if (!__all(pm - m_run <= 8.0f)) {
        const float mn = fmaxf(m_run, pm);
        const float alpha = (m_run == -INFINITY) ? 0.f : exp2_raw(m_run - mn);
        m_run = mn;
        l_run *= alpha;
#pragma unroll
        for (int ds = 0; ds < 4; ++ds)
#pragma unroll
          for (int r = 0; r < 16; ++r) oacc[ds][r] *= alpha;
      }
      float psum = 0.f;
#pragma unroll
      for (int r = 0; r < 16; ++r) {
        const float p0 = exp2_raw(s0[r] - m_run);
        const float p1 = exp2_raw(s1[r] - m_run);
        s0[r] = p0;
        s1[r] = p1;
        psum += p0 + p1;
      }
      psum += __shfl_xor(psum, 32, 64);
      l_run += psum;

#pragma unroll
      for (int sub = 0; sub < 2; ++sub) {
#pragma unroll
        for (int cc = 0; cc < 2; ++cc) {
          const int pb = cc * 8;
          unsigned a0, b0, a1, b1;
          if (sub == 0) {
            a0 = cvt_pk_bf16(s0[pb + 0], s0[pb + 1]);
            b0 = cvt_pk_bf16(s0[pb + 4], s0[pb + 5]);
            a1 = cvt_pk_bf16(s0[pb + 2], s0[pb + 3]);
            b1 = cvt_pk_bf16(s0[pb + 6], s0[pb + 7]);
          } else {
            a0 = cvt_pk_bf16(s1[pb + 0], s1[pb + 1]);
            b0 = cvt_pk_bf16(s1[pb + 4], s1[pb + 5]);
            a1 = cvt_pk_bf16(s1[pb + 2], s1[pb + 3]);
            b1 = cvt_pk_bf16(s1[pb + 6], s1[pb + 7]);
          }
          auto r02 = __builtin_amdgcn_permlane32_swap(a0, b0, false, false);
          auto r13 = __builtin_amdgcn_permlane32_swap(a1, b1, false, false);
          PF f;
          f.u[0] = r02[0];
          f.u[1] = r13[0];
          f.u[2] = r02[1];
          f.u[3] = r13[1];
          pa[sub * 2 + cc] = f;
        }
      }

#pragma unroll
      for (int c = 0; c < 4; ++c) {
#pragma unroll
        for (int ds = 0; ds < 4; ++ds) {
          bf16x8 vf = *reinterpret_cast<const bf16x8*>(
              &vtb[vt_byte(ds * 32 + low, c * 16 + hi * 8)]);
          oacc[ds] = __builtin_amdgcn_mfma_f32_32x32x16_bf16(
              vf, pa[c].v, oacc[ds], 0, 0, 0);
        }
      }
    }
    if (t + 1 < n_tiles) {
      if (have2) v7_wait_vmcnt4(); else v7_wait_vmcnt0();
      V7_TRANSPOSE((t + 1) % V7_RING, LDSVT((t + 1) & 1))
    }
    v7_barrier();
  }

  const float inv_l = 1.0f / l_run;
  u16* orow = out + (long)b * o_sb + (long)h * o_sh + (long)qrow * o_ss;
#pragma unroll
  for (int ds = 0; ds < 4; ++ds) {
#pragma unroll
    for (int g = 0; g < 4; ++g) {
      const int d0 = 8 * g + 4 * hi + 32 * ds;
      const unsigned w0 = cvt_pk_bf16(oacc[ds][4 * g + 0] * inv_l,
                                      oacc[ds][4 * g + 1] * inv_l);
      const unsigned w1 = cvt_pk_bf16(oacc[ds][4 * g + 2] * inv_l,
                                      oacc[ds][4 * g + 3] * inv_l);
      uint2 wv;
      wv.x = w0;
      wv.y = w1;
      *reinterpret_cast<uint2*>(orow + d0) = wv;
    }
  }
  if (hi == 0)
    lse[((long)b * n_heads + h) * S + qrow] =
        m_run * 0.6931471805599453f + __logf(l_run);
}

extern "C" int attn_fwd_v7(void* stream, const void* q, const void* k,
                           const void* v, void* out, void* lse,
                           long q_sb, long q_sh, long q_ss,
                           long k_sb, long k_sh, long k_ss,
                           long v_sb, long v_sh, long v_ss,
                           int batch, int n_heads, int n_kv_heads, int S,
                           float scale) {
  if (S <= 0 || S % 256 != 0 || n_heads % n_kv_heads != 0) return -1;
  launch_fwd_v7(stream, q, k, v, out, lse, q_sb, q_sh, q_ss,
                k_sb, k_sh, k_ss, v_sb, v_sh, v_ss,
                (long)n_heads * S * ATTN_D, (long)S * ATTN_D, ATTN_D,
                batch, n_heads, n_kv_heads, S, scale);
  return 0;
}

extern "C" int attn_fwd_strided(void* stream, const void* q, const void* k,
                                const void* v, void* out, void* lse,
                                const long* st, int batch, int n_heads,
                                int n_kv_heads, int S, float scale) {
  if (S <= 0 || S % 256 != 0 || n_heads <= 0 || batch <= 0 ||
      n_kv_heads <= 0 || n_heads % n_kv_heads != 0)
    return -1;
  if (!st || !attn_strides_ok(st, 12)) return -1;
  launch_fwd_v7(stream, q, k, v, out, lse, st[0], st[1], st[2],
                st[3], st[4], st[5], st[6], st[7], st[8],
                st[9], st[10], st[11], batch, n_heads, n_kv_heads, S, scale);
  return 0;
}


extern "C" int attn_block_fwd(void* stream, const void* q, const void* k,
                              const void* v, void* out, void* lse,
                              const long* st, int batch, int n_heads,
                              int n_kv_heads, int S, float scale,
                              int causal) {
  if (!attn_block_shape_ok(batch, n_heads, n_kv_heads, S)) return -1;
  if (!st || !attn_strides_ok(st, 12)) return -1;
  launch_fwd_v7(stream, q, k, v, out, lse, st[0], st[1], st[2],
                st[3], st[4], st[5], st[6], st[7], st[8],
                st[9], st[10], st[11], batch, n_heads, n_kv_heads, S, scale,
                causal != 0);
  return 0;
}

extern "C" int attn_delta(void* stream, const void* out, const void* dout,
                          void* delta, const long* st, int batch,
                          int n_heads, int S) {
  if (S <= 0 || S % 16 != 0 || n_heads <= 0 || batch <= 0) return -1;
  if (!st || !attn_strides_ok(st, 6)) return -1;
  launch_delta(reinterpret_cast<hipStream_t>(stream), out, dout, delta,
               {st[0], st[1], st[2]}, {st[3], st[4], st[5]},
               batch, n_heads, S);
  return 0;
}

extern "C" int attn_block_bwd(void* stream, const void* q, const void* k,
                              const void* v, const void* dout,
                              const void* lse, const void* delta,
                              void* dq, void* dk, void* dv,
                              const long* st, int batch, int n_heads,
                              int n_kv_heads, int S, float scale,
                              int causal) {
  if (!attn_block_shape_ok(batch, n_heads, n_kv_heads, S)) return -1;
  if (!st || !attn_strides_ok(st, 21)) return -1;
  auto tri = [st](int i) {
    return AttnStride{st[3 * i], st[3 * i + 1], st[3 * i + 2]};
  };
  hipStream_t hs = reinterpret_cast<hipStream_t>(stream);
  if (causal)
    launch_bwd_core<true>(hs, q, k, v, dout, lse, delta, dq, dk, dv,
                          tri(0), tri(1), tri(2), tri(3), tri(4), tri(5),
                          tri(6), batch, n_heads, n_kv_heads, S, scale);
  else
    launch_bwd_core<false>(hs, q, k, v, dout, lse, delta, dq, dk, dv,
                           tri(0), tri(1), tri(2), tri(3), tri(4), tri(5),
                           tri(6), batch, n_heads, n_kv_heads, S, scale);
  return 0;
}


__global__ __launch_bounds__(256) void attn_merge_kernel(
    float* __restrict__ o_acc, float* __restrict__ lse_acc,
    const u16* __restrict__ o_blk, const float* __restrict__ lse_blk,
    long ob_sb, long ob_sh, long ob_ss, int n_heads, int S, long n_rows) {
  const long row = (long)blockIdx.x * 16 + (threadIdx.x >> 4);
  if (row >= n_rows) return;
  const int sub = threadIdx.x & 15;
  float wa = 0.f, wb = 0.f;
  if (sub == 0) {
    const float la = lse_acc[row], lb = lse_blk[row];
    const float m = fmaxf(la, lb);
    if (m != -INFINITY) {
      const float ea = __expf(la - m), eb = __expf(lb - m);
      const float sum = ea + eb;
      wa = ea / sum;
      wb = eb / sum;
      lse_acc[row] = m + __logf(sum);
    }
  }
  wa = __shfl(wa, 0, 16);
  wb = __shfl(wb, 0, 16);
  const long bh = row / S;
  const int s = (int)(row - bh * S);
  const long bi = bh / n_heads;
  const int h = (int)(bh - bi * n_heads);
  union { uint4 u; u16 h[8]; } ob;
  ob.u = *reinterpret_cast<const uint4*>(
      o_blk + bi * ob_sb + (long)h * ob_sh + (long)s * ob_ss + sub * 8);
  float4* acc = reinterpret_cast<float4*>(o_acc + row * ATTN_D + sub * 8);
  float4 a0 = acc[0], a1 = acc[1];
  a0.x = a0.x * wa + bf2f_(ob.h[0]) * wb;
  a0.y = a0.y * wa + bf2f_(ob.h[1]) * wb;
  a0.z = a0.z * wa + bf2f_(ob.h[2]) * wb;
  a0.w = a0.w * wa + bf2f_(ob.h[3]) * wb;
  a1.x = a1.x * wa + bf2f_(ob.h[4]) * wb;
  a1.y = a1.y * wa + bf2f_(ob.h[5]) * wb;
  a1.z = a1.z * wa + bf2f_(ob.h[6]) * wb;
  a1.w = a1.w * wa + bf2f_(ob.h[7]) * wb;
  acc[0] = a0;
  acc[1] = a1;
}

extern "C" int attn_merge(void* stream, void* o_acc, void* lse_acc,
                          const void* o_blk, const void* lse_blk,
                          const long* st, int batch, int n_heads, int S) {
  if (S <= 0 || n_heads <= 0 || batch <= 0) return -1;
  if (!st || !attn_strides_ok(st, 3)) return -1;
  const long n_rows = (long)batch * n_heads * S;
  const long n_blocks = (n_rows + 15) / 16;
  if (n_blocks > 0x7fffffffL) return -1;
  hipLaunchKernelGGL(attn_merge_kernel, dim3((unsigned)n_blocks), dim3(256),
                     0, reinterpret_cast<hipStream_t>(stream),
                     (float*)o_acc, (float*)lse_acc, (const u16*)o_blk,
                     (const float*)lse_blk, st[0], st[1], st[2],
                     n_heads, S, n_rows);
  return 0;
}
```

trainingjob_operator_amd/ops/native.py:

```python
from __future__ import annotations

import ctypes
import os
import subprocess
from typing import Optional

_PKG_DIR = os.path.dirname(os.path.abspath(__file__))
LIB_PATH = os.path.join(_PKG_DIR, "libhipops.so")
SRC_PATH = os.path.join(_PKG_DIR, "hip", "ops.hip")
ATTN_SRC_PATH = os.path.join(_PKG_DIR, "hip", "attention.hip")

_lib: Optional[ctypes.CDLL] = None


class HipOpsUnavailable(RuntimeError):
    pass


def build_ops(verbose: bool = False) -> str:
    cmd = [
        "hipcc", "--offload-arch=gfx950", "-O3", "-std=c++17",
        "-shared", "-fPIC", SRC_PATH, ATTN_SRC_PATH, "-o", LIB_PATH,
    ]
    if verbose:
        print("+", " ".join(cmd))
    subprocess.run(cmd, check=True)
    return LIB_PATH


def _sig(fn, argtypes, restype=None):
    fn.argtypes = argtypes
    fn.restype = restype


def load(require: bool = True) -> Optional[ctypes.CDLL]:
    global _lib
    if _lib is not None:
        return _lib
    if not os.path.exists(LIB_PATH):
        if require:
            raise HipOpsUnavailable(
                f"{LIB_PATH} not built — run trainingjob_operator_amd.ops."
                "native.build_ops() (or __graft_entry__.build())")
        return None
    lib = ctypes.CDLL(LIB_PATH)
    vp, l, i, f = ctypes.c_void_p, ctypes.c_long, ctypes.c_int, ctypes.c_float
    _sig(lib.hipops_arch_check, [], i)
    _sig(lib.rmsnorm_fwd, [vp, vp, vp, vp, vp, vp, vp, l, i, f], i)
    _sig(lib.rmsnorm_bwd, [vp, vp, vp, vp, vp, vp, vp, vp, l, i], i)
    _sig(lib.rmsnorm_bwd_partials, [l, i], l)
    _sig(lib.rmsnorm_dw_reduce, [vp, vp, l, vp, i], i)
    _sig(lib.rope, [vp, vp, vp, vp, l, i, i, i, f], i)
    _sig(lib.rope_at, [vp, vp, vp, vp, l, i, i, i, f, i], i)
    _sig(lib.rope_at_dev, [vp, vp, vp, vp, l, i, i, i, f, vp], i)
    _sig(lib.rope_packed, [vp, vp, vp, vp, l, i, l, l, i, i, f], i)
    _sig(lib.gemv_bf16, [vp, vp, vp, vp, i, i, i], i)
    _sig(lib.gemv_swiglu, [vp, vp, vp, vp, i, i, i], i)
    _sig(lib.gemv_moe_swiglu, [vp, vp, vp, vp, vp, vp, i, i, i, i], i)
    _sig(lib.gemv_moe, [vp, vp, vp, vp, vp, i, i, i, i], i)
    _sig(lib.attn_decode, [vp, vp, vp, vp, vp, vp, vp,
                           i, i, i, i, i, f], i)
    _sig(lib.rope_cache, [vp, vp, vp, vp, vp, vp, vp, i, i, i, i, i], i)
    _sig(lib.swiglu_fwd, [vp, vp, vp, vp, l], i)
    _sig(lib.swiglu_bwd, [vp, vp, vp, vp, vp, vp, l], i)
    _sig(lib.swiglu_packed_fwd, [vp, vp, vp, l, i], i)
    _sig(lib.swiglu_packed_bwd, [vp, vp, vp, vp, l, i], i)
    _sig(lib.ce_fwd, [vp, vp, vp, vp, vp, l, i, i], i)
    _sig(lib.ce_bwd, [vp, vp, vp, vp, vp, vp, l, i, i], i)
    _sig(lib.l2normsq, [vp, vp, l, vp, i, vp], i)
    _sig(lib.rows_gather, [vp, vp, vp, vp, l, i], i)
    _sig(lib.rows_scatter, [vp, vp, vp, vp, l, i], i)
    _sig(lib.rows_scatter_add_f32, [vp, vp, vp, vp, l, i], i)
    _sig(lib.moe_combine, [vp, vp, vp, vp, vp, l, i, i], i)
    _sig(lib.moe_combine_bwd, [vp, vp, vp, vp, vp, vp, vp, l, i, i], i)
    _sig(lib.adamw_step, [vp, vp, vp, vp, vp, vp, vp, l,
                          f, f, f, f, f, f, f, f, f, vp], i)
    _sig(lib.adamw_step_bf16mom, [vp, vp, vp, vp, vp, vp, vp, l,
                                  f, f, f, f, f, f, f, f, f, vp], i)
    _sig(lib.mfma_probe, [vp, vp, vp, vp])
    _sig(lib.attn_fwd, [vp, vp, vp, vp, vp, vp,
                        l, l, l, l, l, l, l, l, l, i, i, i, i, f], i)
    _sig(lib.attn_fwd_v5, [vp, vp, vp, vp, vp, vp,
                           l, l, l, l, l, l, l, l, l, i, i, i, f], i)
    _sig(lib.attn_fwd_nw8, [vp, vp, vp, vp, vp, vp,
                            l, l, l, l, l, l, l, l, l, i, i, i, i, f], i)
    _sig(lib.attn_fwd_v7, [vp, vp, vp, vp, vp, vp,
                           l, l, l, l, l, l, l, l, l, i, i, i, i, f], i)
    _sig(lib.attn_bwd, [vp, vp, vp, vp, vp, vp, vp, vp, vp, vp, vp,
                        l, l, l, l, l, l, l, l, l, i, i, i, i, f], i)
    lp = ctypes.POINTER(ctypes.c_long)
    _sig(lib.attn_fwd_strided, [vp, vp, vp, vp, vp, vp, lp, i, i, i, i, f], i)
    _sig(lib.attn_bwd_strided, [vp, vp, vp, vp, vp, vp, vp, vp, vp, vp, vp,
                                lp, i, i, i, i, f], i)
    _sig(lib.attn_block_fwd, [vp, vp, vp, vp, vp, vp, lp,
                              i, i, i, i, f, i], i)
    _sig(lib.attn_delta, [vp, vp, vp, vp, lp, i, i, i], i)
    _sig(lib.attn_block_bwd, [vp, vp, vp, vp, vp, vp, vp, vp, vp, vp, lp,
                              i, i, i, i, f, i], i)
    _sig(lib.attn_merge, [vp, vp, vp, vp, vp, lp, i, i, i], i)
    _sig(lib.mfma_probe32, [vp, vp, vp, vp])
    assert lib.hipops_arch_check() == 950
    _lib = lib
    return lib


def check_rc(rc: int, op: str, detail: str = "") -> None:
    if rc != 0:
        raise RuntimeError(
            f"hipops {op}: unsupported shape ({detail}) — the kernel "
            f"launcher refused to launch (rc={rc})")


def stride_array(*triples):
    flat = [int(x) for t in triples for x in t]
    assert len(flat) == 3 * len(triples)
    return (ctypes.c_long * len(flat))(*flat)


def available() -> bool:
    return os.path.exists(LIB_PATH)


def stream_ptr() -> ctypes.c_void_p:
    import torch
    return ctypes.c_void_p(torch.cuda.current_stream().cuda_stream)


def tr_probe_maps(device="cuda"):
    import torch
    lib = load()
    lib.tr_probe.argtypes = [ctypes.c_void_p, ctypes.c_void_p,
                             ctypes.c_int, ctypes.c_int]
    results = {}
    for mode in (0, 1, 2, 3):
        out = torch.empty(64, 4, dtype=torch.int16, device=device)
        lib.tr_probe(stream_ptr(), ctypes.c_void_p(out.data_ptr()), 0, mode)
        torch.cuda.synchronize()
        results[mode] = out.to(torch.int32).cpu() & 0xFFFF
    return results
```

Before: 18820 tokens/s.

## Balance attention block scheduling and add optional GQA-split backward with workspace

Flattens the attention forward/backward grids and maps workgroup IDs through a scheduler that orders by causal row rank first and interleaves heads and batches, aiming for better load balance across CUs. Adds an optional split mode for the dK/dV backward kernels that gives each query head its own workgroup, writes fp32 partials to a workspace, and reduces them per KV head in a separate kernel to raise occupancy for GQA. The split path is enabled only through an environment variable and costs extra workspace memory and traffic. The new ordering may change cache locality of K/V across neighbouring workgroups.

```diff
diff --git a/trainingjob_operator_amd/ops/attention.py b/trainingjob_operator_amd/ops/attention.py
--- a/trainingjob_operator_amd/ops/attention.py
+++ b/trainingjob_operator_amd/ops/attention.py
@@ -16,6 +16,14 @@
             and (S % 256 == 0 or (S % 64 == 0 and HKV == H))
             and q.stride(-1) == 1 and k.stride(-1) == 1
             and H % HKV == 0)
+
+
+def _bwd_workspace(lib, B, H, HKV, S, causal, device):
+    nbytes = lib.attn_bwd_ws_bytes(B, H, HKV, S, 1 if causal else 0)
+    if nbytes <= 0:
+        return None, None, 0
+    ws = torch.empty(nbytes, dtype=torch.uint8, device=device)
+    return ws, ws.data_ptr(), nbytes
 
 
 def _run_fwd(q, k, v, scale):
@@ -67,15 +75,16 @@
     dq = torch.empty(B, H, S, D, dtype=torch.bfloat16, device=q.device)
     dk = torch.empty(B, HKV, S, D, dtype=torch.bfloat16, device=q.device)
     dv = torch.empty(B, HKV, S, D, dtype=torch.bfloat16, device=q.device)
-    rc = lib.attn_bwd(
+    ws, ws_ptr, ws_bytes = _bwd_workspace(lib, B, H, HKV, S, True, q.device)
+    rc = lib.attn_bwd_ws(
         native.stream_ptr(), q.data_ptr(), k.data_ptr(), v.data_ptr(),
         out.data_ptr(), dout.data_ptr(), lse.data_ptr(), delta.data_ptr(),
         dq.data_ptr(), dk.data_ptr(), dv.data_ptr(),
         q.stride(0), q.stride(1), q.stride(2),
         k.stride(0), k.stride(1), k.stride(2),
         v.stride(0), v.stride(1), v.stride(2),
-        B, H, HKV, S, scale)
-    native.check_rc(rc, "attn_bwd", f"B={B} H={H} HKV={HKV} S={S}")
+        B, H, HKV, S, scale, ws_ptr, ws_bytes)
+    native.check_rc(rc, "attn_bwd_ws", f"B={B} H={H} HKV={HKV} S={S}")
     return dq, dk, dv
 
 
@@ -149,15 +158,18 @@
         rs, ws, os_ = (_bhsd_strides(R, D, S), _bhsd_strides(W, D, S),
                        _bhsd_strides(H * D, D, S))
         st = native.stride_array(rs, rs, ws, os_, os_, ws, ws, ws)
-        rc = lib.attn_bwd_strided(
+        ws, ws_ptr, ws_bytes = _bwd_workspace(lib, B, H, HKV, S, True,
+                                              qkv.device)
+        rc = lib.attn_bwd_strided_ws(
             native.stream_ptr(), rot.data_ptr(),
             rot.data_ptr() + H * D * esz,
             qkv.data_ptr() + (H + HKV) * D * esz,
             o.data_ptr(), dout.data_ptr(), lse.data_ptr(), delta.data_ptr(),
             dqkv.data_ptr(), dqkv.data_ptr() + H * D * esz,
             dqkv.data_ptr() + (H + HKV) * D * esz,
-            st, B, H, HKV, S, ctx.scale)
-        native.check_rc(rc, "attn_bwd_strided", f"B={B} H={H} HKV={HKV} S={S}")
+            st, B, H, HKV, S, ctx.scale, ws_ptr, ws_bytes)
+        native.check_rc(rc, "attn_bwd_strided_ws",
+                        f"B={B} H={H} HKV={HKV} S={S}")
         _rope_packed(lib, dqkv, dqkv, inv_freq, B * S, H + HKV, W, W, S, D,
                      -1.0)
         return dqkv, None, None, None, None
@@ -339,12 +351,14 @@
     dv = torch.empty(B, HKV, S, 128, dtype=torch.bfloat16, device=q.device)
     st = native.stride_array(_tri(q), _tri(k), _tri(v), _tri(dout),
                              _tri(dq), _tri(dk), _tri(dv))
-    rc = lib.attn_block_bwd(
+    ws, ws_ptr, ws_bytes = _bwd_workspace(lib, B, H, HKV, S, causal,
+                                          q.device)
+    rc = lib.attn_block_bwd_ws(
         native.stream_ptr(), q.data_ptr(), k.data_ptr(), v.data_ptr(),
         dout.data_ptr(), lse.data_ptr(), delta.data_ptr(),
         dq.data_ptr(), dk.data_ptr(), dv.data_ptr(), st,
-        B, H, HKV, S, scale, 1 if causal else 0)
-    native.check_rc(rc, "attn_block_bwd", f"B={B} H={H} HKV={HKV} S={S}")
+        B, H, HKV, S, scale, 1 if causal else 0, ws_ptr, ws_bytes)
+    native.check_rc(rc, "attn_block_bwd_ws", f"B={B} H={H} HKV={HKV} S={S}")
     return dq, dk, dv
 
 
diff --git a/trainingjob_operator_amd/ops/hip/attention.hip b/trainingjob_operator_amd/ops/hip/attention.hip
--- a/trainingjob_operator_amd/ops/hip/attention.hip
+++ b/trainingjob_operator_amd/ops/hip/attention.hip
@@ -2,6 +2,8 @@
 #include <hip/hip_runtime.h>
 #include <hip/hip_bf16.h>
 #include <cstdint>
+#include <cstdlib>
+#include <cstring>
 
 typedef unsigned short u16;
 typedef unsigned int u32;
@@ -36,6 +38,33 @@
 
 __device__ __forceinline__ int p_byte(int row, int col_elem) {
   return (row * ATTN_BN * 2 + col_elem * 2) ^ ((row & 7) << 4);
+}
+
+
+#define ATTN_SCHED_LEGACY 0
+#define ATTN_SCHED_BALANCED 1
+
+struct AttnBlock { int rank, head, batch; };
+
+__host__ __device__ __forceinline__ AttnBlock attn_sched_block(
+    unsigned id, unsigned n_row_blocks, unsigned n_heads, unsigned batch,
+    int sched) {
+  AttnBlock blk;
+  if (sched == ATTN_SCHED_LEGACY) {
+    const unsigned t = id / n_row_blocks;
+    blk.rank = (int)(id - t * n_row_blocks);
+    blk.batch = (int)(t / n_heads);
+    blk.head = (int)(t - (unsigned)blk.batch * n_heads);
+    return blk;
+  }
+  const unsigned M = n_heads * batch;
+  const unsigned r = id / M;
+  const unsigned w = id - r * M;
+  const unsigned p = (M % 8 == 0) ? (w % 8) * (M / 8) + w / 8 : w;
+  blk.rank = (int)r;
+  blk.batch = (int)(p / n_heads);
+  blk.head = (int)(p - (unsigned)blk.batch * n_heads);
+  return blk;
 }
 
 __global__ __launch_bounds__(256) void attn_fwd_kernel(
@@ -487,7 +516,7 @@
     long k_sb, long k_sh, long k_ss,
     long v_sb, long v_sh, long v_ss,
     long o_sb, long o_sh, long o_ss,
-    int n_heads, int gqa_group, int S, float scale2);
+    int n_heads, int gqa_group, int S, float scale2, int batch, int sched);
 
 static inline bool attn_strides_ok(const long* st, int n) {
   for (int i = 0; i < n; ++i)
@@ -495,7 +524,33 @@
   return true;
 }
 
-static void launch_fwd_v7(void* stream, const void* q, const void* k,
+static int attn_sched_mode() {
+  const char* e = std::getenv("AITJ_ATTN_SCHED");
+  if (e && std::strcmp(e, "legacy") == 0) return ATTN_SCHED_LEGACY;
+  return ATTN_SCHED_BALANCED;
+}
+
+extern "C" int attn_sched_decode(int sched, int id, int n_row_blocks,
+                                 int n_heads, int batch, int* rank,
+                                 int* head, int* b) {
+  if (n_row_blocks <= 0 || n_heads <= 0 || batch <= 0 || id < 0 ||
+      (long)id >= (long)n_row_blocks * n_heads * batch ||
+      (sched != ATTN_SCHED_LEGACY && sched != ATTN_SCHED_BALANCED))
+    return -1;
+  const AttnBlock blk = attn_sched_block((unsigned)id, (unsigned)n_row_blocks,
+                                         (unsigned)n_heads, (unsigned)batch,
+                                         sched);
+  *rank = blk.rank;
+  *head = blk.head;
+  *b = blk.batch;
+  return 0;
+}
+
+static inline bool attn_grid_ok(int S, int n_heads, int batch) {
+  return (long)(S / 256) * n_heads * batch <= 0x7fffffffL;
+}
+
+static int launch_fwd_v7(void* stream, const void* q, const void* k,
                           const void* v, void* out, void* lse,
                           long q_sb, long q_sh, long q_ss,
                           long k_sb, long k_sh, long k_ss,
@@ -503,8 +558,9 @@
                           long o_sb, long o_sh, long o_ss,
                           int batch, int n_heads, int n_kv_heads, int S,
                           float scale, bool causal = true) {
+  if (!attn_grid_ok(S, n_heads, batch)) return -1;
   const float scale2 = scale * 1.4426950408889634f;
-  dim3 grid(S / 256, n_heads, batch), block(512);
+  dim3 grid((S / 256) * n_heads * batch), block(512);
   hipLaunchKernelGGL(causal ? attn_fwd_v7_kernel<true>
                             : attn_fwd_v7_kernel<false>, grid, block, 0,
                      reinterpret_cast<hipStream_t>(stream),
@@ -512,7 +568,9 @@
                      (u16*)out, (float*)lse, q_sb, q_sh, q_ss,
                      k_sb, k_sh, k_ss, v_sb, v_sh, v_ss,
                      o_sb, o_sh, o_ss, n_heads,
-                     n_heads / n_kv_heads, S, scale2);
+                     n_heads / n_kv_heads, S, scale2, batch,
+                     attn_sched_mode());
+  return 0;
 }
 
 extern "C" int attn_fwd(void* stream, const void* q, const void* k,
@@ -528,11 +586,10 @@
   if (S % 128 == 0) {
     const float scale2 = scale * 1.4426950408889634f;
     if (S % 256 == 0) {
-      launch_fwd_v7(stream, q, k, v, out, lse, q_sb, q_sh, q_ss,
-                    k_sb, k_sh, k_ss, v_sb, v_sh, v_ss,
-                    (long)n_heads * S * ATTN_D, (long)S * ATTN_D, ATTN_D,
-                    batch, n_heads, n_kv_heads, S, scale);
-      return 0;
+      return launch_fwd_v7(stream, q, k, v, out, lse, q_sb, q_sh, q_ss,
+                           k_sb, k_sh, k_ss, v_sb, v_sh, v_ss,
+                           (long)n_heads * S * ATTN_D, (long)S * ATTN_D,
+                           ATTN_D, batch, n_heads, n_kv_heads, S, scale);
     }
     dim3 grid(S / 128, n_heads, batch), block(256);
     hipLaunchKernelGGL((attn_fwd_v6_kernel<4>), grid, block, 0,
@@ -632,11 +689,13 @@
     long v_sb, long v_sh, long v_ss,
     long do_sb, long do_sh, long do_ss,
     long dq_sb, long dq_sh, long dq_ss,
-    int n_heads, int gqa_group, int S, float scale) {
+    int n_heads, int gqa_group, int S, float scale, int batch, int sched) {
   constexpr int NT = 512;
-  const int qb = gridDim.x - 1 - blockIdx.x;
-  const int h = blockIdx.y;
-  const int b = blockIdx.z;
+  const AttnBlock blk = attn_sched_block(blockIdx.x, S / 256, n_heads, batch,
+                                         sched);
+  const int qb = S / 256 - 1 - blk.rank;
+  const int h = blk.head;
+  const int b = blk.batch;
   const int hkv = h / gqa_group;
   const int tid = threadIdx.x;
   const int wid = tid >> 6;
@@ -827,7 +886,7 @@
 #define BV_LSE_U16 128
 #define BV_BUF_U16 (BV_Q_U16 + BV_DOT_U16 + BV_LSE_U16)
 
-template <bool CAUSAL>
+template <bool CAUSAL, bool SPLIT>
 __global__ __launch_bounds__(512) void attn_bwd_dv_kernel(
     const u16* __restrict__ q, const u16* __restrict__ k,
     const u16* __restrict__ dout, const float* __restrict__ lse,
@@ -836,11 +895,16 @@
     long k_sb, long k_sh, long k_ss,
     long do_sb, long do_sh, long do_ss,
     long dv_sb, long dv_sh, long dv_ss,
-    int n_heads, int n_kv_heads, int S, float scale) {
-  const int kvb = blockIdx.x;
-  const int hkv = blockIdx.y;
-  const int b = blockIdx.z;
+    int n_heads, int n_kv_heads, int S, float scale,
+    float* __restrict__ ws, int batch, int sched) {
+  const AttnBlock blk = attn_sched_block(
+      blockIdx.x, S / 256, SPLIT ? n_heads : n_kv_heads, batch, sched);
+  const int kvb = blk.rank;
   const int gqa_group = n_heads / n_kv_heads;
+  const int hkv = SPLIT ? blk.head / gqa_group : blk.head;
+  const int b = blk.batch;
+  const int g_lo = SPLIT ? blk.head - hkv * gqa_group : 0;
+  const int g_hi = SPLIT ? g_lo + 1 : gqa_group;
   const int tid = threadIdx.x;
   const int wid = tid >> 6;
   const int lane = tid & 63;
@@ -875,7 +939,7 @@
   const int wu64 = __builtin_amdgcn_readfirstlane(tid >> 6);
   uint4 dtst[2];
 
-  for (int g = 0; g < gqa_group; ++g) {
+  for (int g = g_lo; g < g_hi; ++g) {
     const int h = hkv * gqa_group + g;
     const u16* qbase = q + (long)b * q_sb + (long)h * q_sh;
     const u16* dobase = dout + (long)b * do_sb + (long)h * do_sh;
@@ -1007,6 +1071,23 @@
     }
   }
 
+  if (SPLIT) {
+    float* wrow = ws + (((long)b * n_heads + blk.head) * S + kvrow) * ATTN_D;
+#pragma unroll
+    for (int ds = 0; ds < 4; ++ds) {
+#pragma unroll
+      for (int g = 0; g < 4; ++g) {
+        const int d0 = 8 * g + 4 * hi + 32 * ds;
+        float4 wv;
+        wv.x = dvacc[ds][4 * g + 0];
+        wv.y = dvacc[ds][4 * g + 1];
+        wv.z = dvacc[ds][4 * g + 2];
+        wv.w = dvacc[ds][4 * g + 3];
+        *reinterpret_cast<float4*>(wrow + d0) = wv;
+      }
+    }
+    return;
+  }
   u16* dvrow = dv + (long)b * dv_sb + (long)hkv * dv_sh + (long)kvrow * dv_ss;
 #pragma unroll
   for (int ds = 0; ds < 4; ++ds) {
@@ -1033,7 +1114,7 @@
 #define BK_DLT_U16 128
 #define BK_BUF_U16 (BK_Q_U16 + BK_DO_U16 + BK_QT_U16 + BK_LSE_U16 + BK_DLT_U16)
 
-template <bool CAUSAL>
+template <bool CAUSAL, bool SPLIT>
 __global__ __launch_bounds__(512) void attn_bwd_dk_kernel(
     const u16* __restrict__ q, const u16* __restrict__ k,
     const u16* __restrict__ v, const u16* __restrict__ dout,
@@ -1044,11 +1125,16 @@
     long v_sb, long v_sh, long v_ss,
     long do_sb, long do_sh, long do_ss,
     long dk_sb, long dk_sh, long dk_ss,
-    int n_heads, int n_kv_heads, int S, float scale) {
-  const int kvb = blockIdx.x;
-  const int hkv = blockIdx.y;
-  const int b = blockIdx.z;
+    int n_heads, int n_kv_heads, int S, float scale,
+    float* __restrict__ ws, int batch, int sched) {
+  const AttnBlock blk = attn_sched_block(
+      blockIdx.x, S / 256, SPLIT ? n_heads : n_kv_heads, batch, sched);
+  const int kvb = blk.rank;
   const int gqa_group = n_heads / n_kv_heads;
+  const int hkv = SPLIT ? blk.head / gqa_group : blk.head;
+  const int b = blk.batch;
+  const int g_lo = SPLIT ? blk.head - hkv * gqa_group : 0;
+  const int g_hi = SPLIT ? g_lo + 1 : gqa_group;
   const int tid = threadIdx.x;
   const int wid = tid >> 6;
   const int lane = tid & 63;
@@ -1088,7 +1174,7 @@
   const int wu64 = __builtin_amdgcn_readfirstlane(tid >> 6);
   uint4 qtst[2];
 
-  for (int g = 0; g < gqa_group; ++g) {
+  for (int g = g_lo; g < g_hi; ++g) {
     const int h = hkv * gqa_group + g;
     const u16* qbase = q + (long)b * q_sb + (long)h * q_sh;
     const u16* dobase = dout + (long)b * do_sb + (long)h * do_sh;
@@ -1239,6 +1325,23 @@
     }
   }
 
+  if (SPLIT) {
+    float* wrow = ws + (((long)b * n_heads + blk.head) * S + kvrow) * ATTN_D;
+#pragma unroll
+    for (int ds = 0; ds < 4; ++ds) {
+#pragma unroll
+      for (int g = 0; g < 4; ++g) {
+        const int d0 = 8 * g + 4 * hi + 32 * ds;
+        float4 wv;
+        wv.x = dkacc[ds][4 * g + 0];
+        wv.y = dkacc[ds][4 * g + 1];
+        wv.z = dkacc[ds][4 * g + 2];
+        wv.w = dkacc[ds][4 * g + 3];
+        *reinterpret_cast<float4*>(wrow + d0) = wv;
+      }
+    }
+    return;
+  }
   u16* dkrow = dk + (long)b * dk_sb + (long)hkv * dk_sh + (long)kvrow * dk_ss;
 #pragma unroll
   for (int ds = 0; ds < 4; ++ds) {
@@ -1276,6 +1379,70 @@
                      n_heads, S);
 }
 
+
+__global__ __launch_bounds__(256) void attn_bwd_reduce_kernel(
+    const float* __restrict__ ws_k, const float* __restrict__ ws_v,
+    u16* __restrict__ dk, u16* __restrict__ dv,
+    long dk_sb, long dk_sh, long dk_ss,
+    long dv_sb, long dv_sh, long dv_ss,
+    int n_heads, int n_kv_heads, int S, long n_rows) {
+  const long row = (long)blockIdx.x * 16 + (threadIdx.x >> 4);
+  if (row >= n_rows) return;
+  const int sub = threadIdx.x & 15;
+  const int gqa_group = n_heads / n_kv_heads;
+  const long bh = row / S;
+  const int s = (int)(row - bh * S);
+  const long bi = bh / n_kv_heads;
+  const int hkv = (int)(bh - bi * n_kv_heads);
+  const bool is_v = blockIdx.y != 0;
+  const float* src = (is_v ? ws_v : ws_k)
+      + ((bi * n_heads + (long)hkv * gqa_group) * S + s) * ATTN_D + sub * 8;
+  const long hstep = (long)S * ATTN_D;
+  float4 a0 = reinterpret_cast<const float4*>(src)[0];
+  float4 a1 = reinterpret_cast<const float4*>(src)[1];
+  for (int g = 1; g < gqa_group; ++g) {
+    const float4 p0 = reinterpret_cast<const float4*>(src + g * hstep)[0];
+    const float4 p1 = reinterpret_cast<const float4*>(src + g * hstep)[1];
+    a0.x += p0.x; a0.y += p0.y; a0.z += p0.z; a0.w += p0.w;
+    a1.x += p1.x; a1.y += p1.y; a1.z += p1.z; a1.w += p1.w;
+  }
+  uint4 o;
+  o.x = cvt_pk_bf16(a0.x, a0.y);
+  o.y = cvt_pk_bf16(a0.z, a0.w);
+  o.z = cvt_pk_bf16(a1.x, a1.y);
+  o.w = cvt_pk_bf16(a1.z, a1.w);
+  u16* dst = is_v
+      ? dv + bi * dv_sb + (long)hkv * dv_sh + (long)s * dv_ss
+      : dk + bi * dk_sb + (long)hkv * dk_sh + (long)s * dk_ss;
+  *reinterpret_cast<uint4*>(dst + sub * 8) = o;
+}
+
+static inline bool attn_block_shape_ok(int batch, int n_heads,
+                                       int n_kv_heads, int S) {
+  return S > 0 && S % 256 == 0 && n_heads > 0 && batch > 0 &&
+         n_kv_heads > 0 && n_heads % n_kv_heads == 0 &&
+         attn_grid_ok(S, n_heads, batch);
+}
+
+#define ATTN_NUM_CUS 256
+static bool attn_bwd_use_split(int batch, int n_heads, int n_kv_heads, int S,
+                               bool causal) {
+  const char* e = std::getenv("AITJ_ATTN_BWD_SPLIT");
+  if (e && std::strcmp(e, "1") == 0) return true;
+  if (!e || std::strcmp(e, "auto") != 0) return false;
+  if (n_heads == n_kv_heads) return false;
+  const long wgs = (long)batch * n_kv_heads * (S / 256);
+  return wgs < (long)(causal ? 2 : 1) * ATTN_NUM_CUS;
+}
+
+extern "C" long attn_bwd_ws_bytes(int batch, int n_heads, int n_kv_heads,
+                                  int S, int causal) {
+  if (!attn_block_shape_ok(batch, n_heads, n_kv_heads, S)) return 0;
+  if (!attn_bwd_use_split(batch, n_heads, n_kv_heads, S, causal != 0))
+    return 0;
+  return 2L * batch * n_heads * S * ATTN_D * (long)sizeof(float);
+}
+
 template <bool CAUSAL>
 static void launch_bwd_core(hipStream_t st, const void* q, const void* k,
                             const void* v, const void* dout,
@@ -1284,9 +1451,11 @@
                             AttnStride qs, AttnStride ks, AttnStride vs,
                             AttnStride dos, AttnStride dqs, AttnStride dks,
                             AttnStride dvs, int batch, int n_heads,
-                            int n_kv_heads, int S, float scale) {
+                            int n_kv_heads, int S, float scale, void* ws) {
+  const int sched = attn_sched_mode();
+  const int nrb = S / 256;
   {
-    dim3 grid(S / 256, n_heads, batch), block(512);
+    dim3 grid(nrb * n_heads * batch), block(512);
     hipLaunchKernelGGL(attn_bwd_dq_kernel<CAUSAL>, grid, block, 0, st,
                        (const u16*)q, (const u16*)k, (const u16*)v,
                        (const u16*)dout, (const float*)lse,
@@ -1294,49 +1463,102 @@
                        qs.sb, qs.sh, qs.ss, ks.sb, ks.sh, ks.ss,
                        vs.sb, vs.sh, vs.ss, dos.sb, dos.sh, dos.ss,
                        dqs.sb, dqs.sh, dqs.ss,
-                       n_heads, n_heads / n_kv_heads, S, scale);
-  }
-  {
-    dim3 grid(S / 256, n_kv_heads, batch), block(512);
-    hipLaunchKernelGGL(attn_bwd_dv_kernel<CAUSAL>, grid, block, 0, st,
-                       (const u16*)q, (const u16*)k, (const u16*)dout,
-                       (const float*)lse, (u16*)dv,
-                       qs.sb, qs.sh, qs.ss, ks.sb, ks.sh, ks.ss,
-                       dos.sb, dos.sh, dos.ss, dvs.sb, dvs.sh, dvs.ss,
-                       n_heads, n_kv_heads, S, scale);
-    hipLaunchKernelGGL(attn_bwd_dk_kernel<CAUSAL>, grid, block, 0, st,
-                       (const u16*)q, (const u16*)k, (const u16*)v,
-                       (const u16*)dout, (const float*)lse,
-                       (const float*)delta, (u16*)dk,
-                       qs.sb, qs.sh, qs.ss, ks.sb, ks.sh, ks.ss,
-                       vs.sb, vs.sh, vs.ss, dos.sb, dos.sh, dos.ss,
-                       dks.sb, dks.sh, dks.ss,
-                       n_heads, n_kv_heads, S, scale);
-  }
-}
-
-static inline bool attn_block_shape_ok(int batch, int n_heads,
-                                       int n_kv_heads, int S) {
-  return S > 0 && S % 256 == 0 && n_heads > 0 && batch > 0 &&
-         n_kv_heads > 0 && n_heads % n_kv_heads == 0;
-}
-
-static int launch_bwd(void* stream, const void* q, const void* k,
-                      const void* v, const void* out, const void* dout,
-                      const void* lse, void* delta,
-                      void* dq, void* dk, void* dv,
-                      AttnStride qs, AttnStride ks, AttnStride vs,
-                      AttnStride os, AttnStride dos,
-                      AttnStride dqs, AttnStride dks, AttnStride dvs,
-                      int batch, int n_heads, int n_kv_heads, int S,
-                      float scale) {
-  if (!attn_block_shape_ok(batch, n_heads, n_kv_heads, S)) return -1;
-  hipStream_t st = reinterpret_cast<hipStream_t>(stream);
-  launch_delta(st, out, dout, delta, os, dos, batch, n_heads, S);
-  launch_bwd_core<true>(st, q, k, v, dout, lse, delta, dq, dk, dv,
-                        qs, ks, vs, dos, dqs, dks, dvs,
-                        batch, n_heads, n_kv_heads, S, scale);
+                       n_heads, n_heads / n_kv_heads, S, scale, batch, sched);
+  }
+  const bool split = ws != nullptr;
+  float* ws_k = (float*)ws;
+  float* ws_v = split ? ws_k + (long)batch * n_heads * S * ATTN_D : nullptr;
+  dim3 grid(nrb * (split ? n_heads : n_kv_heads) * batch), block(512);
+  auto dv_kernel = split ? attn_bwd_dv_kernel<CAUSAL, true>
+                         : attn_bwd_dv_kernel<CAUSAL, false>;
+  hipLaunchKernelGGL(dv_kernel, grid, block, 0, st,
+                     (const u16*)q, (const u16*)k, (const u16*)dout,
+                     (const float*)lse, (u16*)dv,
+                     qs.sb, qs.sh, qs.ss, ks.sb, ks.sh, ks.ss,
+                     dos.sb, dos.sh, dos.ss, dvs.sb, dvs.sh, dvs.ss,
+                     n_heads, n_kv_heads, S, scale, ws_v, batch, sched);
+  auto dk_kernel = split ? attn_bwd_dk_kernel<CAUSAL, true>
+                         : attn_bwd_dk_kernel<CAUSAL, false>;
+  hipLaunchKernelGGL(dk_kernel, grid, block, 0, st,
+                     (const u16*)q, (const u16*)k, (const u16*)v,
+                     (const u16*)dout, (const float*)lse,
+                     (const float*)delta, (u16*)dk,
+                     qs.sb, qs.sh, qs.ss, ks.sb, ks.sh, ks.ss,
+                     vs.sb, vs.sh, vs.ss, dos.sb, dos.sh, dos.ss,
+                     dks.sb, dks.sh, dks.ss,
+                     n_heads, n_kv_heads, S, scale, ws_k, batch, sched);
+  if (split) {
+    const long n_rows = (long)batch * n_kv_heads * S;
+    hipLaunchKernelGGL(attn_bwd_reduce_kernel,
+                       dim3((unsigned)((n_rows + 15) / 16), 2), dim3(256), 0,
+                       st, (const float*)ws_k, (const float*)ws_v,
+                       (u16*)dk, (u16*)dv, dks.sb, dks.sh, dks.ss,
+                       dvs.sb, dvs.sh, dvs.ss, n_heads, n_kv_heads, S,
+                       n_rows);
+  }
+}
+
+struct AttnBwdArgs {
+  const void *q, *k, *v, *out, *dout, *lse;
+  void *delta, *dq, *dk, *dv;
+  AttnStride qs, ks, vs, os, dos, dqs, dks, dvs;
+  int batch, n_heads, n_kv_heads, S;
+  float scale;
+  bool causal;
+  bool with_delta;
+};
+
+static int launch_bwd_ws(hipStream_t st, const AttnBwdArgs& a, void* ws,
+                         long ws_bytes) {
+  if (!attn_block_shape_ok(a.batch, a.n_heads, a.n_kv_heads, a.S)) return -1;
+  const long need = attn_bwd_ws_bytes(a.batch, a.n_heads, a.n_kv_heads, a.S,
+                                      a.causal);
+  if (need > 0 && (ws == nullptr || ws_bytes < need)) return -2;
+  if (need == 0) ws = nullptr;
+  if (a.with_delta)
+    launch_delta(st, a.out, a.dout, a.delta, a.os, a.dos, a.batch, a.n_heads,
+                 a.S);
+  if (a.causal)
+    launch_bwd_core<true>(st, a.q, a.k, a.v, a.dout, a.lse, a.delta, a.dq,
+                          a.dk, a.dv, a.qs, a.ks, a.vs, a.dos, a.dqs, a.dks,
+                          a.dvs, a.batch, a.n_heads, a.n_kv_heads, a.S,
+                          a.scale, ws);
+  else
+    launch_bwd_core<false>(st, a.q, a.k, a.v, a.dout, a.lse, a.delta, a.dq,
+                           a.dk, a.dv, a.qs, a.ks, a.vs, a.dos, a.dqs, a.dks,
+                           a.dvs, a.batch, a.n_heads, a.n_kv_heads, a.S,
+                           a.scale, ws);
   return 0;
+}
+
+static int launch_bwd_transient(hipStream_t st, const AttnBwdArgs& a) {
+  if (!attn_block_shape_ok(a.batch, a.n_heads, a.n_kv_heads, a.S)) return -1;
+  const long need = attn_bwd_ws_bytes(a.batch, a.n_heads, a.n_kv_heads, a.S,
+                                      a.causal);
+  if (need == 0) return launch_bwd_ws(st, a, nullptr, 0);
+  hipStreamCaptureStatus cs = hipStreamCaptureStatusNone;
+  if (hipStreamIsCapturing(st, &cs) != hipSuccess ||
+      cs != hipStreamCaptureStatusNone)
+    return -3;
+  void* ws = nullptr;
+  if (hipMallocAsync(&ws, (size_t)need, st) != hipSuccess || !ws) return -4;
+  const int rc = launch_bwd_ws(st, a, ws, need);
+  if (hipFreeAsync(ws, st) != hipSuccess) return -5;
+  return rc;
+}
+
+static AttnBwdArgs attn_bwd_dense_args(
+    const void* q, const void* k, const void* v, const void* out,
+    const void* dout, const void* lse, void* delta, void* dq, void* dk,
+    void* dv, long q_sb, long q_sh, long q_ss, long k_sb, long k_sh,
+    long k_ss, long v_sb, long v_sh, long v_ss, int batch, int n_heads,
+    int n_kv_heads, int S, float scale) {
+  const AttnStride dh = attn_dense_stride(n_heads, S);
+  const AttnStride dkv = attn_dense_stride(n_kv_heads, S);
+  return AttnBwdArgs{q, k, v, out, dout, lse, delta, dq, dk, dv,
+                     {q_sb, q_sh, q_ss}, {k_sb, k_sh, k_ss},
+                     {v_sb, v_sh, v_ss}, dh, dh, dh, dkv, dkv,
+                     batch, n_heads, n_kv_heads, S, scale, true, true};
 }
 
 extern "C" int attn_bwd(void* stream, const void* q, const void* k,
@@ -1348,12 +1570,45 @@
                         long v_sb, long v_sh, long v_ss,
                         int batch, int n_heads, int n_kv_heads, int S,
                         float scale) {
-  const AttnStride dh = attn_dense_stride(n_heads, S);
-  const AttnStride dkv = attn_dense_stride(n_kv_heads, S);
-  return launch_bwd(stream, q, k, v, out, dout, lse, delta, dq, dk, dv,
-                    {q_sb, q_sh, q_ss}, {k_sb, k_sh, k_ss},
-                    {v_sb, v_sh, v_ss}, dh, dh, dh, dkv, dkv,
-                    batch, n_heads, n_kv_heads, S, scale);
+  return launch_bwd_transient(
+      reinterpret_cast<hipStream_t>(stream),
+      attn_bwd_dense_args(q, k, v, out, dout, lse, delta, dq, dk, dv,
+                          q_sb, q_sh, q_ss, k_sb, k_sh, k_ss,
+                          v_sb, v_sh, v_ss, batch, n_heads, n_kv_heads, S,
+                          scale));
+}
+
+extern "C" int attn_bwd_ws(void* stream, const void* q, const void* k,
+                           const void* v, const void* out, const void* dout,
+                           const void* lse, void* delta,
+                           void* dq, void* dk, void* dv,
+                           long q_sb, long q_sh, long q_ss,
+                           long k_sb, long k_sh, long k_ss,
+                           long v_sb, long v_sh, long v_ss,
+                           int batch, int n_heads, int n_kv_heads, int S,
+                           float scale, void* ws, long ws_bytes) {
+  return launch_bwd_ws(
+      reinterpret_cast<hipStream_t>(stream),
+      attn_bwd_dense_args(q, k, v, out, dout, lse, delta, dq, dk, dv,
+                          q_sb, q_sh, q_ss, k_sb, k_sh, k_ss,
+                          v_sb, v_sh, v_ss, batch, n_heads, n_kv_heads, S,
+                          scale),
+      ws, ws_bytes);
+}
+
+static bool attn_bwd_strided_args(
+    AttnBwdArgs* a, const void* q, const void* k, const void* v,
+    const void* out, const void* dout, const void* lse, void* delta,
+    void* dq, void* dk, void* dv, const long* st, int batch, int n_heads,
+    int n_kv_heads, int S, float scale) {
+  if (!st || !attn_strides_ok(st, 24)) return false;
+  auto tri = [st](int i) {
+    return AttnStride{st[3 * i], st[3 * i + 1], st[3 * i + 2]};
+  };
+  *a = AttnBwdArgs{q, k, v, out, dout, lse, delta, dq, dk, dv,
+                   tri(0), tri(1), tri(2), tri(3), tri(4), tri(5), tri(6),
+                   tri(7), batch, n_heads, n_kv_heads, S, scale, true, true};
+  return true;
 }
 
 extern "C" int attn_bwd_strided(void* stream, const void* q, const void* k,
@@ -1362,13 +1617,26 @@
                                 void* delta, void* dq, void* dk, void* dv,
                                 const long* st, int batch, int n_heads,
                                 int n_kv_heads, int S, float scale) {
-  if (!st || !attn_strides_ok(st, 24)) return -1;
-  auto tri = [st](int i) {
-    return AttnStride{st[3 * i], st[3 * i + 1], st[3 * i + 2]};
-  };
-  return launch_bwd(stream, q, k, v, out, dout, lse, delta, dq, dk, dv,
-                    tri(0), tri(1), tri(2), tri(3), tri(4), tri(5), tri(6),
-                    tri(7), batch, n_heads, n_kv_heads, S, scale);
+  AttnBwdArgs a;
+  if (!attn_bwd_strided_args(&a, q, k, v, out, dout, lse, delta, dq, dk, dv,
+                             st, batch, n_heads, n_kv_heads, S, scale))
+    return -1;
+  return launch_bwd_transient(reinterpret_cast<hipStream_t>(stream), a);
+}
+
+extern "C" int attn_bwd_strided_ws(void* stream, const void* q, const void* k,
+                                   const void* v, const void* out,
+                                   const void* dout, const void* lse,
+                                   void* delta, void* dq, void* dk, void* dv,
+                                   const long* st, int batch, int n_heads,
+                                   int n_kv_heads, int S, float scale,
+                                   void* ws, long ws_bytes) {
+  AttnBwdArgs a;
+  if (!attn_bwd_strided_args(&a, q, k, v, out, dout, lse, delta, dq, dk, dv,
+                             st, batch, n_heads, n_kv_heads, S, scale))
+    return -1;
+  return launch_bwd_ws(reinterpret_cast<hipStream_t>(stream), a, ws,
+                       ws_bytes);
 }
 
 
@@ -1381,11 +1649,13 @@
     long k_sb, long k_sh, long k_ss,
     long v_sb, long v_sh, long v_ss,
     long o_sb, long o_sh, long o_ss,
-    int n_heads, int gqa_group, int S, float scale2) {
+    int n_heads, int gqa_group, int S, float scale2, int batch, int sched) {
   constexpr int NT = 512;
-  const int qb = gridDim.x - 1 - blockIdx.x;
-  const int h = blockIdx.y;
-  const int b = blockIdx.z;
+  const AttnBlock blk = attn_sched_block(blockIdx.x, S / 256, n_heads, batch,
+                                         sched);
+  const int qb = S / 256 - 1 - blk.rank;
+  const int h = blk.head;
+  const int b = blk.batch;
   const int hkv = h / gqa_group;
   const int tid = threadIdx.x;
   const int wid = tid >> 6;
@@ -1616,11 +1886,10 @@
                            int batch, int n_heads, int n_kv_heads, int S,
                            float scale) {
   if (S <= 0 || S % 256 != 0 || n_heads % n_kv_heads != 0) return -1;
-  launch_fwd_v7(stream, q, k, v, out, lse, q_sb, q_sh, q_ss,
-                k_sb, k_sh, k_ss, v_sb, v_sh, v_ss,
-                (long)n_heads * S * ATTN_D, (long)S * ATTN_D, ATTN_D,
-                batch, n_heads, n_kv_heads, S, scale);
-  return 0;
+  return launch_fwd_v7(stream, q, k, v, out, lse, q_sb, q_sh, q_ss,
+                       k_sb, k_sh, k_ss, v_sb, v_sh, v_ss,
+                       (long)n_heads * S * ATTN_D, (long)S * ATTN_D, ATTN_D,
+                       batch, n_heads, n_kv_heads, S, scale);
 }
 
 extern "C" int attn_fwd_strided(void* stream, const void* q, const void* k,
@@ -1631,10 +1900,9 @@
       n_kv_heads <= 0 || n_heads % n_kv_heads != 0)
     return -1;
   if (!st || !attn_strides_ok(st, 12)) return -1;
-  launch_fwd_v7(stream, q, k, v, out, lse, st[0], st[1], st[2],
-                st[3], st[4], st[5], st[6], st[7], st[8],
-                st[9], st[10], st[11], batch, n_heads, n_kv_heads, S, scale);
-  return 0;
+  return launch_fwd_v7(stream, q, k, v, out, lse, st[0], st[1], st[2],
+                       st[3], st[4], st[5], st[6], st[7], st[8], st[9],
+                       st[10], st[11], batch, n_heads, n_kv_heads, S, scale);
 }
 
 
@@ -1645,11 +1913,10 @@
                               int causal) {
   if (!attn_block_shape_ok(batch, n_heads, n_kv_heads, S)) return -1;
   if (!st || !attn_strides_ok(st, 12)) return -1;
-  launch_fwd_v7(stream, q, k, v, out, lse, st[0], st[1], st[2],
-                st[3], st[4], st[5], st[6], st[7], st[8],
-                st[9], st[10], st[11], batch, n_heads, n_kv_heads, S, scale,
-                causal != 0);
-  return 0;
+  return launch_fwd_v7(stream, q, k, v, out, lse, st[0], st[1], st[2],
+                       st[3], st[4], st[5], st[6], st[7], st[8], st[9],
+                       st[10], st[11], batch, n_heads, n_kv_heads, S, scale,
+                       causal != 0);
 }
 
 extern "C" int attn_delta(void* stream, const void* out, const void* dout,
@@ -1663,6 +1930,22 @@
   return 0;
 }
 
+static bool attn_block_bwd_args(
+    AttnBwdArgs* a, const void* q, const void* k, const void* v,
+    const void* dout, const void* lse, const void* delta, void* dq, void* dk,
+    void* dv, const long* st, int batch, int n_heads, int n_kv_heads, int S,
+    float scale, int causal) {
+  if (!st || !attn_strides_ok(st, 21)) return false;
+  auto tri = [st](int i) {
+    return AttnStride{st[3 * i], st[3 * i + 1], st[3 * i + 2]};
+  };
+  *a = AttnBwdArgs{q, k, v, nullptr, dout, lse, const_cast<void*>(delta),
+                   dq, dk, dv, tri(0), tri(1), tri(2), AttnStride{0, 0, 0},
+                   tri(3), tri(4), tri(5), tri(6), batch, n_heads,
+                   n_kv_heads, S, scale, causal != 0, false};
+  return true;
+}
+
 extern "C" int attn_block_bwd(void* stream, const void* q, const void* k,
                               const void* v, const void* dout,
                               const void* lse, const void* delta,
@@ -1670,21 +1953,26 @@
                               const long* st, int batch, int n_heads,
                               int n_kv_heads, int S, float scale,
                               int causal) {
-  if (!attn_block_shape_ok(batch, n_heads, n_kv_heads, S)) return -1;
-  if (!st || !attn_strides_ok(st, 21)) return -1;
-  auto tri = [st](int i) {
-    return AttnStride{st[3 * i], st[3 * i + 1], st[3 * i + 2]};
-  };
-  hipStream_t hs = reinterpret_cast<hipStream_t>(stream);
-  if (causal)
-    launch_bwd_core<true>(hs, q, k, v, dout, lse, delta, dq, dk, dv,
-                          tri(0), tri(1), tri(2), tri(3), tri(4), tri(5),
-                          tri(6), batch, n_heads, n_kv_heads, S, scale);
-  else
-    launch_bwd_core<false>(hs, q, k, v, dout, lse, delta, dq, dk, dv,
-                           tri(0), tri(1), tri(2), tri(3), tri(4), tri(5),
-                           tri(6), batch, n_heads, n_kv_heads, S, scale);
-  return 0;
+  AttnBwdArgs a;
+  if (!attn_block_bwd_args(&a, q, k, v, dout, lse, delta, dq, dk, dv, st,
+                           batch, n_heads, n_kv_heads, S, scale, causal))
+    return -1;
+  return launch_bwd_transient(reinterpret_cast<hipStream_t>(stream), a);
+}
+
+extern "C" int attn_block_bwd_ws(void* stream, const void* q, const void* k,
+                                 const void* v, const void* dout,
+                                 const void* lse, const void* delta,
+                                 void* dq, void* dk, void* dv,
+                                 const long* st, int batch, int n_heads,
+                                 int n_kv_heads, int S, float scale,
+                                 int causal, void* ws, long ws_bytes) {
+  AttnBwdArgs a;
+  if (!attn_block_bwd_args(&a, q, k, v, dout, lse, delta, dq, dk, dv, st,
+                           batch, n_heads, n_kv_heads, S, scale, causal))
+    return -1;
+  return launch_bwd_ws(reinterpret_cast<hipStream_t>(stream), a, ws,
+                       ws_bytes);
 }
 
 
diff --git a/trainingjob_operator_amd/ops/native.py b/trainingjob_operator_amd/ops/native.py
--- a/trainingjob_operator_amd/ops/native.py
+++ b/trainingjob_operator_amd/ops/native.py
@@ -98,6 +98,16 @@
     _sig(lib.attn_block_bwd, [vp, vp, vp, vp, vp, vp, vp, vp, vp, vp, lp,
                               i, i, i, i, f, i], i)
     _sig(lib.attn_merge, [vp, vp, vp, vp, vp, lp, i, i, i], i)
+    _sig(lib.attn_bwd_ws_bytes, [i, i, i, i, i], l)
+    _sig(lib.attn_bwd_ws, [vp, vp, vp, vp, vp, vp, vp, vp, vp, vp, vp,
+                           l, l, l, l, l, l, l, l, l, i, i, i, i, f,
+                           vp, l], i)
+    _sig(lib.attn_bwd_strided_ws, [vp, vp, vp, vp, vp, vp, vp, vp, vp, vp,
+                                   vp, lp, i, i, i, i, f, vp, l], i)
+    _sig(lib.attn_block_bwd_ws, [vp, vp, vp, vp, vp, vp, vp, vp, vp, vp, lp,
+                                 i, i, i, i, f, i, vp, l], i)
+    ip = ctypes.POINTER(ctypes.c_int)
+    _sig(lib.attn_sched_decode, [i, i, i, i, i, ip, ip, ip], i)
     _sig(lib.mfma_probe32, [vp, vp, vp, vp])
     assert lib.hipops_arch_check() == 950
     _lib = lib
```

Measured after the change: 20000 tokens/s, median of 6. 6.3% higher.
